# debbiemarkslab/EVcouplings

Measured on NVIDIA H100. Metric: PLM gradient evals/s as N*L^2*q cell-ops/s, higher is better.
Workload: dtype f32 parameters/accumulation; tensor-core products as bf16 hi+lo pairs (16 mantissa bits)

## Files before the change

### evcouplings_b200/_lib.py

```python
import ctypes
import os

_HERE = os.path.dirname(os.path.abspath(__file__))
LIB_PATH = os.path.join(_HERE, "csrc", "libevcplm.so")
ABI_VERSION = 2


class EngineUnavailableError(RuntimeError):
    """libevcplm.so (the sm_90a CUDA engine) is missing / unloadable / has no device."""


class EngineError(RuntimeError):
    """A libevcplm call returned non-zero."""


c_void_p = ctypes.c_void_p
c_i32 = ctypes.c_int32
c_i64 = ctypes.c_int64
c_f32 = ctypes.c_float
c_f64 = ctypes.c_double


class FitParams(ctypes.Structure):
    _fields_ = [("max_iterations", c_i32), ("m", c_i32), ("epsilon", c_f32), ("lambda_h", c_f32),
                ("lambda_J", c_f32), ("max_linesearch", c_i32), ("min_step", c_f64), ("max_step", c_f64),
                ("ftol", c_f64), ("gtol", c_f64), ("xtol", c_f64), ("precision_schedule", c_i32),
                ("switch_factor", c_f32)]


class FitResult(ctypes.Structure):
    _fields_ = [("status", c_i32), ("iterations", c_i32), ("evaluations", c_i32), ("switched_at", c_i32),
                ("fx", c_f64), ("negloglk", c_f64), ("seconds", c_f64)]


class FitState(ctypes.Structure):
    _fields_ = [("version", c_i32), ("returning", c_i32), ("status", c_i32), ("k", c_i32), ("evaluations", c_i32),
                ("m", c_i32), ("hist", c_i32), ("end", c_i32), ("low", c_i32), ("switched_at", c_i32),
                ("n", c_i64), ("fx", c_f64), ("negloglk", c_f64), ("xnorm", c_f64), ("gnorm", c_f64),
                ("ys", c_f64 * 32), ("yy", c_f64), ("seconds", c_f64)]


FIT_STATE_VERSION = 1
FIT_VEC_X, FIT_VEC_G, FIT_VEC_S, FIT_VEC_Y = 0, 1, 2, 3

ALLREDUCE_CB = ctypes.CFUNCTYPE(ctypes.c_int, ctypes.c_void_p, ctypes.c_void_p, c_i64, ctypes.c_void_p)
PROGRESS_CB = ctypes.CFUNCTYPE(ctypes.c_int, ctypes.c_void_p, c_i32, c_f64, c_f64, c_f64, c_f64, c_i32, c_f64,
                               c_f64, c_f64)
CHECKPOINT_CB = ctypes.CFUNCTYPE(ctypes.c_int, ctypes.c_void_p, ctypes.POINTER(FitState), ctypes.c_void_p)

LBFGS_STATUS = {
    0: "LBFGS_SUCCESS", 2: "LBFGS_ALREADY_MINIMIZED", -1021: "LBFGSERR_CANCELED",
    -1000: "LBFGSERR_INVALIDPARAMETERS", -1001: "LBFGSERR_MINIMUMSTEP", -1002: "LBFGSERR_MAXIMUMSTEP",
    -1003: "LBFGSERR_MAXIMUMLINESEARCH", -1004: "LBFGSERR_MAXIMUMITERATION", -1005: "LBFGSERR_WIDTHTOOSMALL",
    -1006: "LBFGSERR_ROUNDING_ERROR", -1007: "LBFGSERR_INCREASEGRADIENT",
}

PROTOTYPES = {
    "evc_abi_version": (ctypes.c_int, []),
    "evc_last_error": (ctypes.c_char_p, []),
    "evc_device_count": (ctypes.c_int, []),
    "evc_device_info": (ctypes.c_int, [c_i32, c_void_p, c_void_p, c_void_p, c_void_p]),
    "evc_hamming_counts": (ctypes.c_int, [c_void_p, c_i64, c_i32, c_i32, c_i32, c_void_p]),
    "evc_hamming_plane_words": (c_i64, [c_i64, c_i32]),
    "evc_hamming_num_tiles": (c_i64, [c_i64]),
    "evc_hamming_pack": (ctypes.c_int, [c_void_p, c_i64, c_i32, c_void_p, c_void_p]),
    "evc_hamming_count_tiles": (ctypes.c_int, [c_void_p, c_i64, c_i32, c_i32, c_i64, c_i64, c_void_p, c_void_p]),
    "evc_hamming_counts_mult": (ctypes.c_int, [c_void_p, c_void_p, c_i64, c_i32, c_i32, c_i32, c_void_p]),
    "evc_hamming_count_tiles_mult": (ctypes.c_int, [c_void_p, c_void_p, c_i64, c_i32, c_i32, c_i64, c_i64, c_void_p,
                                                    c_void_p]),
    "evc_msa_unique": (ctypes.c_int, [c_void_p, c_i64, c_i32, c_void_p, c_void_p, c_void_p, c_void_p, c_void_p]),
    "evc_msa_unique_host": (ctypes.c_int, [c_void_p, c_i64, c_i32, c_i32, c_void_p, c_void_p, c_void_p, c_void_p]),
    "evc_a2m_scan": (ctypes.c_int, [ctypes.c_char_p, c_void_p, c_void_p, c_void_p]),
    "evc_a2m_read": (ctypes.c_int, [ctypes.c_char_p, c_i64, c_i64, c_void_p, c_void_p, c_i64]),
    "evc_msa_encode": (ctypes.c_int, [c_void_p, c_i64, c_i64, c_void_p, c_void_p, c_i64, c_void_p, c_void_p, c_void_p]),
    "evc_identities_to_seq": (ctypes.c_int, [c_void_p, c_void_p, c_i64, c_i32, c_void_p, c_void_p]),
    "evc_plm_create": (ctypes.c_int, [c_void_p, c_void_p, c_i64, c_i32, c_i32, c_i32, c_void_p, c_i32]),
    "evc_plm_create_alphabet": (ctypes.c_int, [c_void_p, c_void_p, c_i64, c_i32, c_i32, c_i32, c_void_p, c_i32]),
    "evc_plm_destroy": (None, [c_void_p]),
    "evc_plm_num_params": (c_i64, [c_void_p]),
    "evc_plm_eval_data": (ctypes.c_int, [c_void_p, c_void_p, c_void_p, c_void_p, c_void_p]),
    "evc_plm_set_backward": (ctypes.c_int, [c_void_p, c_i32]),
    "evc_plm_set_forward": (ctypes.c_int, [c_void_p, c_i32]),
    "evc_plm_set_precision": (ctypes.c_int, [c_void_p, c_i32]),
    "evc_plm_set_seq_chunk": (ctypes.c_int, [c_void_p, c_i64]),
    "evc_plm_tc_bytes": (ctypes.c_int, [c_i64, c_i32, c_i32, c_i32, c_i64, c_i32, c_void_p]),
    "evc_plm_tc_bytes_alphabet": (ctypes.c_int, [c_i64, c_i32, c_i32, c_i32, c_i64, c_i32, c_void_p]),
    "evc_plm_device_bytes": (c_i64, [c_void_p]),
    "evc_fit_workspace_bytes": (c_i64, [c_i64, c_i32]),
    "evc_plm_set_host_history": (ctypes.c_int, [c_void_p, c_i32]),
    "evc_fit_workspace_split_bytes": (ctypes.c_int, [c_i64, c_i32, c_i32, c_void_p, c_void_p]),
    "evc_plm_host_bytes": (ctypes.c_int, [c_void_p, c_void_p, c_void_p]),
    "evc_fit_default_params": (None, [c_void_p]),
    "evc_plm_fit": (ctypes.c_int, [c_void_p, c_void_p, c_void_p, c_void_p, c_void_p, c_void_p, c_void_p, c_void_p,
                                   c_void_p]),
    "evc_plm_fit_checkpointed": (ctypes.c_int, [c_void_p, c_void_p, c_void_p, c_void_p, c_void_p, c_void_p, c_void_p,
                                                c_void_p, c_void_p, c_f64, c_void_p, c_void_p, c_void_p]),
    "evc_plm_fit_prepare": (ctypes.c_int, [c_void_p, c_i32]),
    "evc_plm_fit_vector": (ctypes.c_int, [c_void_p, c_i32, c_i32, c_void_p]),
    "evc_plm_pack_fx": (ctypes.c_int, [c_void_p, c_void_p, c_void_p]),
    "evc_plm_unpack_fx": (ctypes.c_int, [c_void_p, c_void_p, c_void_p]),
    "evc_plm_set_profiling": (ctypes.c_int, [c_void_p, c_i32]),
    "evc_plm_last_stage_ms": (ctypes.c_int, [c_void_p, c_void_p]),
    "evc_plm_add_regulariser": (ctypes.c_int, [c_void_p, c_void_p, c_void_p, c_void_p, c_f32, c_f32, c_void_p]),
    "evc_plm_eval_host": (ctypes.c_int, [c_void_p, c_void_p, c_void_p, c_void_p, c_f32, c_f32]),
    "evc_plm_weighted_counts": (ctypes.c_int, [c_void_p, c_void_p, c_void_p, c_void_p]),
    "evc_vec_dot": (ctypes.c_int, [c_void_p, c_void_p, c_i64, c_void_p, c_void_p]),
    "evc_vec_axpby": (ctypes.c_int, [c_void_p, c_void_p, c_f32, c_f32, c_i64, c_void_p]),
    "evc_vec_copy": (ctypes.c_int, [c_void_p, c_void_p, c_i64, c_void_p]),
    "evc_vec_sub": (ctypes.c_int, [c_void_p, c_void_p, c_void_p, c_i64, c_void_p]),
    "evc_vec_checksum": (ctypes.c_int, [c_void_p, c_i64, c_void_p, c_void_p]),
    "evc_lbfgs_direction": (ctypes.c_int, [c_void_p, c_void_p, c_void_p, c_void_p, c_void_p, c_void_p,
                                           c_i64, c_i32, c_i32, c_i32, c_void_p]),
    "evc_lbfgs_update_pair": (ctypes.c_int, [c_void_p, c_void_p, c_void_p, c_void_p, c_void_p, c_void_p,
                                             c_void_p, c_void_p, c_i64, c_void_p]),
    "evc_ec_scores": (ctypes.c_int, [c_void_p, c_void_p, c_void_p, c_i32, c_i32, c_void_p, c_void_p, c_void_p, c_void_p]),
    "evc_plm_energies": (ctypes.c_int, [c_void_p, c_void_p, c_void_p, c_void_p]),
    "evc_fn_scores": (ctypes.c_int, [c_void_p, c_i32, c_i32, c_void_p, c_void_p]),
}

_lib = None


def load():
    global _lib
    if _lib is not None:
        return _lib
    if not os.path.exists(LIB_PATH):
        raise EngineUnavailableError(
            "CUDA engine library not built: %s is missing. There is no CPU fallback; "
            "build it with evcouplings_b200/csrc/build.sh (nvcc, sm_90a)." % LIB_PATH)
    try:
        lib = ctypes.CDLL(LIB_PATH)
    except OSError as e:
        raise EngineUnavailableError("cannot load %s: %s" % (LIB_PATH, e))
    for name, (restype, argtypes) in PROTOTYPES.items():
        try:
            fn = getattr(lib, name)
        except AttributeError:
            raise EngineUnavailableError("%s does not export %s" % (LIB_PATH, name))
        fn.restype = restype
        fn.argtypes = argtypes
    if lib.evc_abi_version() != ABI_VERSION:
        raise EngineUnavailableError("libevcplm ABI version mismatch")
    _lib = lib
    return lib


def check(rc, what=""):
    if rc != 0:
        msg = load().evc_last_error()
        raise EngineError("%s failed: %s" % (what or "libevcplm call", msg.decode() if msg else "unknown error"))


def require_device():
    lib = load()
    n = lib.evc_device_count()
    if n <= 0:
        raise EngineUnavailableError(
            "libevcplm found no CUDA device; the PLM engine has no CPU fallback")
    return n
```

### evcouplings_b200/csrc/api.cu

```cuda
#include "../../include/evcplm.h"

#include <stdlib.h>

#include <algorithm>
#include <new>
#include <string>
#include <vector>

#include "common.cuh"
#include "internal.h"

namespace evc {
static thread_local std::string g_err;
void set_error(const std::string &msg) { g_err = msg; }
}

using namespace evc;

static cudaStream_t as_stream(void *s) { return reinterpret_cast<cudaStream_t>(s); }

static const char SUPPORTED_Q[] =
    "supported: 2 <= q <= 32 states with the gap as a state, 2 <= q <= 31 with the ignored gap coded q; "
    "every code must be below 32, the 5 bit-planes of the Hamming pass";

static int require_gather_q(const evc_plm *h, const char *what)
{
    if (plm_gather_supported_q(h->g.q)) return 0;
    set_error(std::string(what) + ": the gather kernels support q in {4, 5, 20, 21} only, this handle has q=" +
              std::to_string(h->g.q) + "; select the tensor-core path with evc_plm_set_forward(h, 1)");
    return 1;
}

static void plm_geom_init(PlmGeom &g, int64_t N, int L, int q, int gap_code)
{
    g.N = N;
    g.L = L;
    g.Lp = (int)round_up(L, 4);
    g.q = q;
    g.gap_code = gap_code;
    g.QB = gap_code >= 0 ? q + 1 : q;
    g.S = (q % 2) ? q : q + 1;
    g.Nr = round_up(N, PLM_BWD_TS);
    g.Nld = round_up(N, 32);
    g.L4 = g.Lp / 4;
    g.ntiles_f = (int)ceil_div(N, PLM_FWD_TS);
    g.ntiles_b = (int)ceil_div(N, PLM_BWD_TS);
    g.n_params = (int64_t)L * q + (int64_t)L * (L - 1) / 2 * q * q;
}
struct HandleBytes {
    size_t codes, msa4, wts;
    explicit HandleBytes(const PlmGeom &g)
        : codes((size_t)g.N * g.L), msa4((size_t)g.L4 * g.Nld * sizeof(uint32_t)), wts((size_t)g.N * sizeof(float)) {}
};
struct TcBwdBytes {
    size_t xt, rt, gd;
    explicit TcBwdBytes(const PlmTcGeom &t)
        : xt((size_t)t.Mp * t.Kp * 2), rt((size_t)t.Np * t.Kp * 2), gd((size_t)t.planes * t.Mp * t.Np * sizeof(float)) {}
};
struct TcFwdBytes {
    size_t x, wt, zt, gh_part, fx_part;
    TcFwdBytes(const PlmGeom &g, const PlmTcfGeom &t)
        : x((size_t)t.Xrows * t.Kw * 2), wt((size_t)t.Mp * t.Kw * 2), zt((size_t)t.Mp * t.Ns * sizeof(float)),
          gh_part((size_t)g.L * t.ntiles_s * g.S * sizeof(float)), fx_part((size_t)g.L * t.ntiles_s * sizeof(double)) {}
};

template <class T>
static bool dalloc(evc_plm *h, T **p, size_t bytes)
{
    if (cudaMalloc(p, bytes) != cudaSuccess) return false;
    h->bytes += (int64_t)bytes;
    return true;
}

extern "C" {

int evc_abi_version(void) { return EVCPLM_ABI_VERSION; }

const char *evc_last_error(void) { return g_err.c_str(); }

int evc_device_count(void)
{
    int n = 0;
    if (cudaGetDeviceCount(&n) != cudaSuccess) {
        set_error("cudaGetDeviceCount failed (no CUDA device / driver?)");
        return -1;
    }
    return n;
}

int evc_device_info(int32_t device, int32_t *sm_count, int32_t *cc_major, int32_t *cc_minor,
                    int64_t *total_mem_bytes)
{
    cudaDeviceProp p;
    EVC_CUDA(cudaGetDeviceProperties(&p, device));
    if (sm_count) *sm_count = p.multiProcessorCount;
    if (cc_major) *cc_major = p.major;
    if (cc_minor) *cc_minor = p.minor;
    if (total_mem_bytes) *total_mem_bytes = (int64_t)p.totalGlobalMem;
    return 0;
}

int64_t evc_hamming_plane_words(int64_t N, int32_t L) { return hamming_plane_words(N, L); }
int64_t evc_hamming_num_tiles(int64_t N) { return hamming_num_tiles(N); }

int evc_hamming_pack(const uint8_t *d_codes, int64_t N, int32_t L, uint32_t *d_planes, void *stream)
{
    return hamming_pack(d_codes, N, L, d_planes, as_stream(stream));
}

int evc_hamming_count_tiles(const uint32_t *d_planes, int64_t N, int32_t L, int32_t min_identical,
                            int64_t tile_begin, int64_t tile_end, int32_t *d_counts, void *stream)
{
    return hamming_count_tiles(d_planes, nullptr, N, L, min_identical, tile_begin, tile_end, d_counts,
                               as_stream(stream));
}

int evc_hamming_count_tiles_mult(const uint32_t *d_planes, const int32_t *d_mult, int64_t N, int32_t L,
                                 int32_t min_identical, int64_t tile_begin, int64_t tile_end, int32_t *d_counts,
                                 void *stream)
{
    if (!d_mult) { set_error("evc_hamming_count_tiles_mult: null multiplicities"); return 1; }
    return hamming_count_tiles(d_planes, d_mult, N, L, min_identical, tile_begin, tile_end, d_counts,
                               as_stream(stream));
}

static int hamming_counts_host(const char *fn, const uint8_t *codes, const int32_t *mult, int64_t N, int32_t L,
                               int32_t min_identical, int32_t device, int32_t *counts_out)
{
    const std::string name(fn);
    if (!codes || !counts_out || N <= 0 || L <= 0) {
        set_error(name + ": empty alignment or null pointer");
        return 1;
    }
    {
        unsigned mx = 0;
        const size_t total = (size_t)N * L;
        for (size_t e = 0; e < total; e++) mx = codes[e] > mx ? codes[e] : mx;
        if (mx >= 32) {
            set_error(name + ": sequence code " + std::to_string(mx) + " out of range (codes must be < 32)");
            return 1;
        }
    }
    if (mult) {
        int64_t sum = 0;
        for (int64_t r = 0; r < N; r++) {
            if (mult[r] < 1) { set_error(name + ": multiplicities must be >= 1"); return 1; }
            sum += mult[r];
        }
        if (sum > INT32_MAX) { set_error(name + ": the multiplicities sum to more than 2^31 - 1"); return 1; }
    }
    EVC_CUDA(cudaSetDevice(device));
    uint8_t *d_codes = nullptr;
    uint32_t *d_planes = nullptr;
    int32_t *d_counts = nullptr, *d_mult = nullptr;
    int rc = 1;
    do {
        if (cudaMalloc(&d_codes, (size_t)N * L) != cudaSuccess ||
            cudaMalloc(&d_planes, (size_t)hamming_plane_words(N, L) * sizeof(uint32_t)) != cudaSuccess ||
            cudaMalloc(&d_counts, (size_t)N * sizeof(int32_t)) != cudaSuccess ||
            (mult && cudaMalloc(&d_mult, (size_t)N * sizeof(int32_t)) != cudaSuccess)) {
            set_error(name + ": device allocation failed");
            break;
        }
        if (cudaMemcpy(d_codes, codes, (size_t)N * L, cudaMemcpyHostToDevice) != cudaSuccess ||
            (mult && cudaMemcpy(d_mult, mult, (size_t)N * sizeof(int32_t), cudaMemcpyHostToDevice) != cudaSuccess) ||
            cudaMemset(d_counts, 0, (size_t)N * sizeof(int32_t)) != cudaSuccess) {
            set_error(name + ": H2D failed");
            break;
        }
        if (hamming_pack(d_codes, N, L, d_planes, 0)) break;
        if (hamming_count_tiles(d_planes, d_mult, N, L, min_identical, 0, hamming_num_tiles(N), d_counts, 0)) break;
        if (cudaMemcpy(counts_out, d_counts, (size_t)N * sizeof(int32_t), cudaMemcpyDeviceToHost) !=
            cudaSuccess) {
            set_error(name + ": kernel/D2H failed: " + cudaGetErrorString(cudaGetLastError()));
            break;
        }
        rc = 0;
    } while (0);
    cudaFree(d_codes);
    cudaFree(d_planes);
    cudaFree(d_counts);
    cudaFree(d_mult);
    return rc;
}

int evc_hamming_counts(const uint8_t *codes, int64_t N, int32_t L, int32_t min_identical, int32_t device,
                       int32_t *counts_out)
{
    return hamming_counts_host("evc_hamming_counts", codes, nullptr, N, L, min_identical, device, counts_out);
}

int evc_hamming_counts_mult(const uint8_t *codes, const int32_t *mult, int64_t N, int32_t L, int32_t min_identical,
                            int32_t device, int32_t *counts_out)
{
    if (!mult) { set_error("evc_hamming_counts_mult: null multiplicities"); return 1; }
    return hamming_counts_host("evc_hamming_counts_mult", codes, mult, N, L, min_identical, device, counts_out);
}

int evc_msa_unique(const uint8_t *d_codes, int64_t N, int32_t L, int32_t *d_first, int32_t *d_inverse,
                   int32_t *d_mult, int64_t *U_out, void *stream)
{
    if (!d_codes || !d_first || !d_inverse || !d_mult || !U_out) {
        set_error("evc_msa_unique: null pointer");
        return 1;
    }
    return msa_unique(d_codes, N, L, d_first, d_inverse, d_mult, U_out, as_stream(stream));
}

int evc_msa_unique_host(const uint8_t *codes, int64_t N, int32_t L, int32_t device, int32_t *first_out,
                        int32_t *inverse_out, int32_t *mult_out, int64_t *U_out)
{
    if (!codes || !first_out || !inverse_out || !mult_out || !U_out || N <= 0 || L <= 0) {
        set_error("evc_msa_unique_host: empty alignment or null pointer");
        return 1;
    }
    EVC_CUDA(cudaSetDevice(device));
    uint8_t *d_codes = nullptr;
    int32_t *d_idx = nullptr;
    int rc = 1;
    do {
        if (cudaMalloc(&d_codes, (size_t)N * L) != cudaSuccess ||
            cudaMalloc(&d_idx, (size_t)3 * N * sizeof(int32_t)) != cudaSuccess) {
            set_error("evc_msa_unique_host: device allocation failed");
            break;
        }
        if (cudaMemcpy(d_codes, codes, (size_t)N * L, cudaMemcpyHostToDevice) != cudaSuccess) {
            set_error("evc_msa_unique_host: H2D failed");
            break;
        }
        int64_t U = 0;
        if (msa_unique(d_codes, N, L, d_idx, d_idx + N, d_idx + 2 * N, &U, 0)) break;
        if (cudaMemcpy(first_out, d_idx, (size_t)U * sizeof(int32_t), cudaMemcpyDeviceToHost) != cudaSuccess ||
            cudaMemcpy(inverse_out, d_idx + N, (size_t)N * sizeof(int32_t), cudaMemcpyDeviceToHost) != cudaSuccess ||
            cudaMemcpy(mult_out, d_idx + 2 * N, (size_t)U * sizeof(int32_t), cudaMemcpyDeviceToHost) != cudaSuccess) {
            set_error(std::string("evc_msa_unique_host: D2H failed: ") + cudaGetErrorString(cudaGetLastError()));
            break;
        }
        *U_out = U;
        rc = 0;
    } while (0);
    cudaFree(d_codes);
    cudaFree(d_idx);
    return rc;
}

int evc_identities_to_seq(const uint8_t *d_codes, const uint8_t *d_seq, int64_t N, int32_t L, int32_t *d_out,
                          void *stream)
{
    if (!d_codes || !d_seq || !d_out) { set_error("evc_identities_to_seq: null pointer"); return 1; }
    return identities_to_seq(d_codes, d_seq, N, L, d_out, as_stream(stream));
}

void evc_plm_destroy(evc_plm_t *h)
{
    if (!h) return;
    cudaSetDevice(h->device);
    cudaFree(h->d_codes);
    cudaFree(h->d_msa4);
    cudaFree(h->d_perm);
    cudaFree(h->d_bstart);
    cudaFree(h->d_wts);
    cudaFree(h->d_W);
    cudaFree(h->d_G);
    cudaFree(h->d_R);
    cudaFree(h->d_gh_part);
    cudaFree(h->d_fx_part);
    cudaFree(h->d_x_tmp);
    cudaFree(h->d_g_tmp);
    cudaFree(h->d_fx_tmp);
    cudaFree(h->d_xt);
    cudaFree(h->d_rt_hi);
    cudaFree(h->d_rt_lo);
    cudaFree(h->d_Gd);
    free(h->tc_maps);
    cudaFree(h->d_x1h);
    cudaFree(h->d_wt_hi);
    cudaFree(h->d_wt_lo);
    cudaFree(h->d_zt);
    cudaFree(h->d_gh_part2);
    cudaFree(h->d_fx_part2);
    free(h->tcf_maps);
    cudaFree(h->d_wp_hi);
    cudaFree(h->d_wp_lo);
    cudaFree(h->d_gh_part3);
    cudaFree(h->d_fx_part3);
    free(h->tcff_maps);
    for (int k = 0; k < 6; k++)
        if (h->ev[k]) cudaEventDestroy(h->ev[k]);
    fit_work_free(h->fit);
    delete h;
}

static int plm_create(const char *fn, bool any_q, evc_plm_t **out, const uint8_t *codes, int64_t N, int32_t L,
                      int32_t q, int32_t gap_code, const float *weights, int32_t device)
{
    const std::string name(fn);
    if (!out || !codes || !weights) { set_error(name + ": null pointer"); return 1; }
    *out = nullptr;
    if (N <= 0 || L < 2) { set_error(name + ": need N >= 1 sequences and L >= 2 sites"); return 1; }
    if (!any_q && !plm_gather_supported_q(q)) {
        set_error(name + ": unsupported number of states q=" + std::to_string(q) +
                  " (supported: 4, 5, 20, 21; evc_plm_create_alphabet takes 2 <= q <= 32)");
        return 1;
    }
    if (gap_code >= 0 && gap_code != q) {
        set_error(name + ": gap_code must be -1 or q");
        return 1;
    }
    if (!plm_supported_q(q, gap_code)) {
        set_error(name + ": unsupported number of states q=" + std::to_string(q) +
                  (gap_code >= 0 ? " with the ignored gap" : "") + " (" + SUPPORTED_Q + ")");
        return 1;
    }
    if (L > 65535) { set_error(name + ": L too large"); return 1; }
    {
        unsigned mx = 0;
        const size_t total = (size_t)N * L;
        for (size_t e = 0; e < total; e++) mx = codes[e] > mx ? codes[e] : mx;
        if ((int)mx >= (gap_code >= 0 ? q + 1 : q)) {
            set_error(name + ": sequence code " + std::to_string(mx) + " out of range (valid: 0.." +
                      std::to_string((gap_code >= 0 ? q + 1 : q) - 1) + (gap_code >= 0 ? ", the last one being the ignored gap)" : ")"));
            return 1;
        }
    }
    EVC_CUDA(cudaSetDevice(device));
    evc_plm *h = new (std::nothrow) evc_plm();
    if (!h) { set_error(name + ": out of host memory"); return 1; }
    h->device = device;
    PlmGeom &g = h->g;
    plm_geom_init(g, N, L, q, gap_code);
    const HandleBytes hb(g);

    bool ok = dalloc(h, &h->d_codes, hb.codes) && dalloc(h, &h->d_msa4, hb.msa4) && dalloc(h, &h->d_wts, hb.wts);
    if (!ok) {
        set_error(name + ": device allocation failed: " +
                  cudaGetErrorString(cudaGetLastError()));
        evc_plm_destroy(h);
        return 1;
    }
    ok = cudaMemcpy(h->d_codes, codes, (size_t)N * L, cudaMemcpyHostToDevice) == cudaSuccess &&
         cudaMemcpy(h->d_wts, weights, (size_t)N * sizeof(float), cudaMemcpyHostToDevice) == cudaSuccess;
    if (!ok || plm_pack_msa(g, h->d_codes, h->d_msa4, 0) || cudaDeviceSynchronize() != cudaSuccess) {
        if (ok) set_error(name + ": packing failed: " + cudaGetErrorString(cudaGetLastError()));
        else set_error(name + ": H2D failed");
        evc_plm_destroy(h);
        return 1;
    }
    *out = h;
    return 0;
}

int evc_plm_create(evc_plm_t **out, const uint8_t *codes, int64_t N, int32_t L, int32_t q, int32_t gap_code,
                   const float *weights, int32_t device)
{
    return plm_create("evc_plm_create", false, out, codes, N, L, q, gap_code, weights, device);
}

int evc_plm_create_alphabet(evc_plm_t **out, const uint8_t *codes, int64_t N, int32_t L, int32_t q, int32_t gap_code,
                            const float *weights, int32_t device)
{
    return plm_create("evc_plm_create_alphabet", true, out, codes, N, L, q, gap_code, weights, device);
}

static int ensure_expanded(evc_plm *h)
{
    if (h->expanded_ready) return 0;
    EVC_CUDA(cudaSetDevice(h->device));
    const PlmGeom &g = h->g;
    const size_t w_bytes = (size_t)g.w_floats() * sizeof(float);
    const size_t r_bytes = (size_t)g.L * g.Nr * g.S * sizeof(float);
    if (!dalloc(h, &h->d_W, w_bytes) || !dalloc(h, &h->d_R, r_bytes)) {
        set_error(std::string("libevcplm: device allocation of the expanded couplings failed: ") +
                  cudaGetErrorString(cudaGetLastError()));
        return 1;
    }
    EVC_CUDA(cudaMemset(h->d_W, 0, w_bytes));
    EVC_CUDA(cudaMemset(h->d_R, 0, r_bytes));
    h->expanded_ready = true;
    return 0;
}

static int ensure_gather(evc_plm *h)
{
    if (h->gather_ready) return 0;
    if (require_gather_q(h, "libevcplm")) return 1;
    if (ensure_expanded(h)) return 1;
    const PlmGeom &g = h->g;
    const size_t w_bytes = (size_t)g.w_floats() * sizeof(float);
    const bool ok = dalloc(h, &h->d_perm, (size_t)g.ntiles_b * g.L * PLM_BWD_CAP * sizeof(uint32_t)) &&
                    dalloc(h, &h->d_bstart, (size_t)g.ntiles_b * g.L * PLM_BWD_BS * sizeof(uint16_t)) &&
                    dalloc(h, &h->d_G, w_bytes) &&
                    dalloc(h, &h->d_gh_part, (size_t)g.L * g.ntiles_f * g.S * sizeof(float)) &&
                    dalloc(h, &h->d_fx_part, (size_t)g.L * g.ntiles_f * sizeof(double));
    if (!ok) {
        set_error(std::string("libevcplm: device allocation of the gather-path buffers failed: ") +
                  cudaGetErrorString(cudaGetLastError()));
        return 1;
    }
    if (plm_build_buckets(g, h->d_codes, h->d_perm, h->d_bstart, 0)) return 1;
    EVC_CUDA(cudaDeviceSynchronize());
    h->gather_ready = true;
    return 0;
}

int64_t evc_plm_num_params(const evc_plm_t *h) { return h ? h->g.n_params : -1; }

int evc_plm_set_precision(evc_plm_t *h, int32_t mode)
{
    if (!h) { set_error("evc_plm_set_precision: null handle"); return 1; }
    if (mode != 0 && mode != 1) {
        set_error("evc_plm_set_precision: mode must be 0 (fp32-equivalent, bf16 hi+lo products) or 1 (bf16 tiles)");
        return 1;
    }
    h->precision = mode;
    return 0;
}

int evc_plm_eval_data(evc_plm_t *h, const float *d_x, float *d_g, double *d_fx, void *stream)
{
    if (!h || !d_x || !d_g || !d_fx) { set_error("evc_plm_eval_data: null pointer"); return 1; }
    cudaStream_t st = as_stream(stream);
    const PlmGeom &g = h->g;
    const bool prof = h->profiling;
    const bool tc = h->bwd_mode == 1;
    const bool tcf = h->fwd_mode == 1;
    const bool tcff = h->fwd_mode == 2;
    const int single = h->precision == 1 ? 1 : 0;
    void *rt_lo = single ? nullptr : h->d_rt_lo;
    float *gJ = d_g + (int64_t)g.L * g.q;
    if (tc && h->tc.n_chunks > 1) {
        if (!tcf) {
            set_error("evc_plm_eval_data: sequence chunks need the tensor-core forward (evc_plm_set_forward 1)");
            return 1;
        }
        h->ev_valid = false;
        if (plm_tcf_expand(g, h->tcf, d_x, h->d_wt_hi, h->d_wt_lo, single, st)) return 1;
        for (int c = 0; c < h->tc.n_chunks; c++) {
            const int64_t n0 = (int64_t)c * h->tc.C, nreal = std::min(h->tc.C, g.N - n0);
            if (plm_tcf_build_x(g, h->tcf, h->d_msa4, h->d_x1h, n0, st)) return 1;
            if (plm_tc_build_xt(g, h->tc, h->d_msa4, h->d_xt, n0, st)) return 1;
            if (plm_tcf_logits(g, h->tcf, h->tcf_maps, h->d_zt, single, nreal, st)) return 1;
            if (plm_tcf_softmax(g, h->tcf, h->d_zt, d_x, h->d_msa4, h->d_wts, h->d_rt_hi, rt_lo, h->tc.Kp,
                                h->d_gh_part2, h->d_fx_part2, n0, nreal, st))
                return 1;
            if (plm_tc_backward(g, h->tc, h->tc_maps, h->d_Gd, single, c, st)) return 1;
        }
        if (plm_tc_finalize_pairs(g, h->tc, h->d_Gd, h->tc.planes, gJ, 1.0f, st)) return 1;
        return plm_finalize_fields_n(g, h->d_gh_part2, h->d_fx_part2, d_g, d_fx, h->tcf.ntiles_s, st);
    }
    if (!tc || (!tcf && !tcff)) {
        if (require_gather_q(h, "evc_plm_eval_data") || ensure_gather(h)) return 1;
    }
    if (prof) EVC_CUDA(cudaEventRecord(h->ev[0], st));
    if (tcff) {
        if (plm_tcff_expand(g, h->tcff, d_x, h->d_wp_hi, h->d_wp_lo, single, st)) return 1;
        if (prof) EVC_CUDA(cudaEventRecord(h->ev[1], st));
        if (plm_tcff_forward(g, h->tcff, h->tcff_maps, d_x, h->d_msa4, h->d_wts, h->d_rt_hi, h->d_rt_lo, h->tc.Kp,
                             h->d_gh_part3, h->d_fx_part3, single, st))
            return 1;
        if (prof) {
            EVC_CUDA(cudaEventRecord(h->ev[2], st));
            EVC_CUDA(cudaEventRecord(h->ev[3], st));
        }
        if (plm_tc_backward(g, h->tc, h->tc_maps, h->d_Gd, single, 0, st)) return 1;
        if (prof) EVC_CUDA(cudaEventRecord(h->ev[4], st));
        if (plm_tc_finalize_pairs(g, h->tc, h->d_Gd, h->tc.planes, gJ, 1.0f, st)) return 1;
        if (plm_finalize_fields_n(g, h->d_gh_part3, h->d_fx_part3, d_g, d_fx, h->tcff.ntile_part, st)) return 1;
    } else if (tcf) {
        if (plm_tcf_expand(g, h->tcf, d_x, h->d_wt_hi, h->d_wt_lo, single, st)) return 1;
        if (prof) EVC_CUDA(cudaEventRecord(h->ev[1], st));
        if (plm_tcf_logits(g, h->tcf, h->tcf_maps, h->d_zt, single, g.N, st)) return 1;
        if (prof) EVC_CUDA(cudaEventRecord(h->ev[2], st));
        if (plm_tcf_softmax(g, h->tcf, h->d_zt, d_x, h->d_msa4, h->d_wts, h->d_rt_hi, rt_lo, h->tc.Kp,
                            h->d_gh_part2, h->d_fx_part2, 0, g.N, st))
            return 1;
        if (prof) EVC_CUDA(cudaEventRecord(h->ev[3], st));
        if (plm_tc_backward(g, h->tc, h->tc_maps, h->d_Gd, single, 0, st)) return 1;
        if (prof) EVC_CUDA(cudaEventRecord(h->ev[4], st));
        if (plm_tc_finalize_pairs(g, h->tc, h->d_Gd, h->tc.planes, gJ, 1.0f, st)) return 1;
        if (plm_finalize_fields_n(g, h->d_gh_part2, h->d_fx_part2, d_g, d_fx, h->tcf.ntiles_s, st)) return 1;
    } else {
        if (plm_expand(g, d_x, h->d_W, st)) return 1;
        if (!tc) EVC_CUDA(cudaMemsetAsync(h->d_G, 0, (size_t)g.w_floats() * sizeof(float), st));
        if (prof) EVC_CUDA(cudaEventRecord(h->ev[1], st));
        if (plm_forward(g, h->d_W, d_x, h->d_msa4, h->d_wts, h->d_R, tc ? h->d_rt_hi : nullptr,
                        tc ? h->d_rt_lo : nullptr, h->tc.Kp, h->d_gh_part, h->d_fx_part, st))
            return 1;
        if (prof) {
            EVC_CUDA(cudaEventRecord(h->ev[2], st));
            EVC_CUDA(cudaEventRecord(h->ev[3], st));
        }
        if (tc) {
            if (plm_tc_backward(g, h->tc, h->tc_maps, h->d_Gd, single, 0, st)) return 1;
            if (prof) EVC_CUDA(cudaEventRecord(h->ev[4], st));
            if (plm_tc_finalize_pairs(g, h->tc, h->d_Gd, h->tc.planes, gJ, 1.0f, st)) return 1;
            if (plm_finalize_fields(g, h->d_gh_part, h->d_fx_part, d_g, d_fx, st)) return 1;
        } else {
            if (plm_backward(g, h->d_R, h->d_perm, h->d_bstart, h->d_G, st)) return 1;
            if (prof) EVC_CUDA(cudaEventRecord(h->ev[4], st));
            if (plm_finalize(g, h->d_G, h->d_gh_part, h->d_fx_part, d_g, gJ, d_fx, 1.0f, st)) return 1;
        }
    }
    if (prof) {
        EVC_CUDA(cudaEventRecord(h->ev[5], st));
        h->ev_valid = true;
    }
    return 0;
}

int evc_plm_set_backward(evc_plm_t *h, int32_t mode)
{
    if (!h) { set_error("evc_plm_set_backward: null handle"); return 1; }
    if (mode != 0 && mode != 1) { set_error("evc_plm_set_backward: mode must be 0 (gather) or 1 (tensor core)"); return 1; }
    if (mode == 0 && require_gather_q(h, "evc_plm_set_backward")) return 1;
    EVC_CUDA(cudaSetDevice(h->device));
    if (mode == 1 && !h->d_xt) {
        int sm_count = 0;
        EVC_CUDA(cudaDeviceGetAttribute(&sm_count, cudaDevAttrMultiProcessorCount, h->device));
        plm_tc_geometry(h->g, sm_count, h->seq_chunk, h->tc);
        const PlmTcGeom &t = h->tc;
        const TcBwdBytes b(t);
        if (!dalloc(h, &h->d_xt, b.xt) || !dalloc(h, &h->d_rt_hi, b.rt) || !dalloc(h, &h->d_rt_lo, b.rt) ||
            !dalloc(h, &h->d_Gd, b.gd)) {
            set_error(std::string("evc_plm_set_backward: device allocation failed: ") +
                      cudaGetErrorString(cudaGetLastError()));
            return 1;
        }
        EVC_CUDA(cudaMemset(h->d_xt, 0, b.xt));
        EVC_CUDA(cudaMemset(h->d_rt_hi, 0, b.rt));
        EVC_CUDA(cudaMemset(h->d_rt_lo, 0, b.rt));
        EVC_CUDA(cudaMemset(h->d_Gd, 0, b.gd));
        if (t.n_chunks == 1 && plm_tc_build_xt(h->g, t, h->d_msa4, h->d_xt, 0, 0)) return 1;
        EVC_CUDA(cudaDeviceSynchronize());
        h->tc_maps = aligned_alloc(64, round_up((int64_t)plm_tc_map_bytes(), 64));
        if (!h->tc_maps) { set_error("evc_plm_set_backward: out of host memory"); return 1; }
        if (plm_tc_make_maps(t, h->d_xt, h->d_rt_hi, h->d_rt_lo, h->tc_maps)) return 1;
    }
    h->bwd_mode = mode;
    return 0;
}

int evc_plm_set_forward(evc_plm_t *h, int32_t mode)
{
    if (!h) { set_error("evc_plm_set_forward: null handle"); return 1; }
    if (mode < 0 || mode > 2) {
        set_error("evc_plm_set_forward: mode must be 0 (gather), 1 (tensor core) or 2 (tensor core, fused softmax)");
        return 1;
    }
    if (mode == 0 && require_gather_q(h, "evc_plm_set_forward")) return 1;
    EVC_CUDA(cudaSetDevice(h->device));
    const int64_t chunk = plm_seq_chunk_round(h->seq_chunk);
    const bool chunked = chunk > 0 && chunk < h->g.N;
    if (mode == 2 && (!plm_tcff_supported(h->g) || (int64_t)h->g.L * h->g.q > 8192 || chunked)) mode = 1;
    if (mode >= 1) {
        if (evc_plm_set_backward(h, 1)) return 1;
        if (!h->d_x1h) {
            plm_tcf_geometry(h->g, h->tc, h->tcf);
            const PlmTcfGeom &t = h->tcf;
            const TcFwdBytes b(h->g, t);
            if (!dalloc(h, &h->d_x1h, b.x)) {
                set_error("evc_plm_set_forward: device allocation failed (one-hot operand)");
                return 1;
            }
            EVC_CUDA(cudaMemset(h->d_x1h, 0, b.x));
            if (h->tc.n_chunks == 1 && plm_tcf_build_x(h->g, t, h->d_msa4, h->d_x1h, 0, 0)) return 1;
            EVC_CUDA(cudaDeviceSynchronize());
        }
    }
    if (mode == 1 && !h->d_zt) {
        const PlmTcfGeom &t = h->tcf;
        const TcFwdBytes b(h->g, t);
        if (!dalloc(h, &h->d_wt_hi, b.wt) || !dalloc(h, &h->d_wt_lo, b.wt) || !dalloc(h, &h->d_zt, b.zt) ||
            !dalloc(h, &h->d_gh_part2, b.gh_part) || !dalloc(h, &h->d_fx_part2, b.fx_part)) {
            set_error(std::string("evc_plm_set_forward: device allocation failed: ") +
                      cudaGetErrorString(cudaGetLastError()));
            return 1;
        }
        EVC_CUDA(cudaMemset(h->d_wt_hi, 0, b.wt));
        EVC_CUDA(cudaMemset(h->d_wt_lo, 0, b.wt));
        h->tcf_maps = aligned_alloc(64, round_up((int64_t)plm_tc_map_bytes(), 64));
        if (!h->tcf_maps) { set_error("evc_plm_set_forward: out of host memory"); return 1; }
        if (plm_tcf_make_maps(t, h->d_wt_hi, h->d_wt_lo, h->d_x1h, h->tcf_maps)) return 1;
    }
    if (mode == 2 && !h->d_wp_hi) {
        plm_tcff_geometry(h->g, h->tcff);
        const PlmTcffGeom &t = h->tcff;
        const size_t wb = (size_t)t.Np * t.Kw * 2;
        if (!dalloc(h, &h->d_wp_hi, wb) || !dalloc(h, &h->d_wp_lo, wb) ||
            !dalloc(h, &h->d_gh_part3, (size_t)h->g.L * t.ntile_part * h->g.S * sizeof(float)) ||
            !dalloc(h, &h->d_fx_part3, (size_t)h->g.L * t.ntile_part * sizeof(double))) {
            set_error(std::string("evc_plm_set_forward: device allocation failed: ") +
                      cudaGetErrorString(cudaGetLastError()));
            return 1;
        }
        EVC_CUDA(cudaMemset(h->d_wp_hi, 0, wb));
        EVC_CUDA(cudaMemset(h->d_wp_lo, 0, wb));
        h->tcff_maps = aligned_alloc(64, round_up((int64_t)plm_tc_map_bytes(), 64));
        if (!h->tcff_maps) { set_error("evc_plm_set_forward: out of host memory"); return 1; }
        if (plm_tcff_make_maps(t, h->d_x1h, h->d_wp_hi, h->d_wp_lo, h->tcff_maps)) return 1;
    }
    h->fwd_mode = mode;
    return 0;
}

int evc_plm_set_seq_chunk(evc_plm_t *h, int64_t seq_chunk)
{
    if (!h) { set_error("evc_plm_set_seq_chunk: null handle"); return 1; }
    if (seq_chunk < 0) { set_error("evc_plm_set_seq_chunk: seq_chunk must be >= 0 (0: whole shard)"); return 1; }
    const int64_t c = plm_seq_chunk_round(seq_chunk);
    if (h->d_xt) {
        const int64_t have = h->tc.n_chunks > 1 ? h->tc.C : 0;
        const int64_t want = (c > 0 && c < h->g.N) ? c : 0;
        if (have != want) {
            set_error("evc_plm_set_seq_chunk: the tensor-core buffers already exist for " +
                      (have ? std::to_string(have) + " sequences per chunk" : std::string("the whole shard")) +
                      "; set the chunk before evc_plm_set_backward / evc_plm_set_forward");
            return 1;
        }
    }
    h->seq_chunk = c;
    return 0;
}

static int plm_tc_bytes(const char *fn, bool any_q, int64_t N, int32_t L, int32_t q, int32_t gap_code,
                        int64_t seq_chunk, int32_t sm_count, int64_t *bytes_out)
{
    const std::string name(fn);
    if (!bytes_out) { set_error(name + ": null pointer"); return 1; }
    const bool q_ok = any_q ? plm_supported_q(q, gap_code) : plm_gather_supported_q(q);
    if (N <= 0 || L < 2 || L > 65535 || !q_ok || (gap_code >= 0 && gap_code != q) || seq_chunk < 0 ||
        sm_count <= 0) {
        set_error(name + ": invalid arguments (need N >= 1, 2 <= L <= 65535, gap_code -1 or q, seq_chunk >= 0, "
                  "sm_count >= 1; q: " + (any_q ? std::string(SUPPORTED_Q)
                                                : std::string("4, 5, 20 or 21; evc_plm_tc_bytes_alphabet takes "
                                                              "2 <= q <= 32")) + ")");
        return 1;
    }
    PlmGeom g{};
    plm_geom_init(g, N, L, q, gap_code);
    PlmTcGeom t{};
    plm_tc_geometry(g, sm_count, seq_chunk, t);
    PlmTcfGeom f{};
    plm_tcf_geometry(g, t, f);
    const HandleBytes hb(g);
    const TcBwdBytes bb(t);
    const TcFwdBytes fb(g, f);
    *bytes_out = (int64_t)(hb.codes + hb.msa4 + hb.wts + bb.xt + 2 * bb.rt + bb.gd + fb.x + 2 * fb.wt + fb.zt +
                           fb.gh_part + fb.fx_part);
    return 0;
}

int evc_plm_tc_bytes(int64_t N, int32_t L, int32_t q, int32_t gap_code, int64_t seq_chunk, int32_t sm_count,
                     int64_t *bytes_out)
{
    return plm_tc_bytes("evc_plm_tc_bytes", false, N, L, q, gap_code, seq_chunk, sm_count, bytes_out);
}

int evc_plm_tc_bytes_alphabet(int64_t N, int32_t L, int32_t q, int32_t gap_code, int64_t seq_chunk,
                              int32_t sm_count, int64_t *bytes_out)
{
    return plm_tc_bytes("evc_plm_tc_bytes_alphabet", true, N, L, q, gap_code, seq_chunk, sm_count, bytes_out);
}

int64_t evc_plm_device_bytes(const evc_plm_t *h) { return h ? h->bytes + fit_work_bytes(h->fit) : -1; }

int64_t evc_fit_workspace_bytes(int64_t n, int32_t m) { return n > 0 && m > 0 ? fit_work_bytes(n, m) : -1; }

int evc_fit_workspace_split_bytes(int64_t n, int32_t m, int32_t host_pairs, int64_t *device_bytes,
                                  int64_t *host_bytes)
{
    if (!device_bytes || !host_bytes) { set_error("evc_fit_workspace_split_bytes: null pointer"); return 1; }
    if (n <= 0 || m < 1 || m > 32 || host_pairs < 0 || host_pairs > m) {
        set_error("evc_fit_workspace_split_bytes: invalid arguments (need n >= 1, 1 <= m <= 32, "
                  "0 <= host_pairs <= m)");
        return 1;
    }
    fit_work_bytes(n, m, host_pairs, device_bytes, host_bytes);
    return 0;
}

int evc_plm_set_host_history(evc_plm_t *h, int32_t host_pairs)
{
    if (!h) { set_error("evc_plm_set_host_history: null handle"); return 1; }
    if (host_pairs < 0 || host_pairs > 32) {
        set_error("evc_plm_set_host_history: host_pairs must be in 0..32");
        return 1;
    }
    h->host_pairs = host_pairs;
    return 0;
}

int evc_plm_host_bytes(const evc_plm_t *h, int64_t *bytes_out, double *pin_seconds_out)
{
    if (!h || !bytes_out) { set_error("evc_plm_host_bytes: null pointer"); return 1; }
    *bytes_out = fit_work_host_bytes(h->fit);
    if (pin_seconds_out) *pin_seconds_out = fit_work_pin_seconds(h->fit);
    return 0;
}

int evc_plm_set_profiling(evc_plm_t *h, int32_t enable)
{
    if (!h) { set_error("evc_plm_set_profiling: null handle"); return 1; }
    EVC_CUDA(cudaSetDevice(h->device));
    if (enable && !h->ev[0])
        for (int k = 0; k < 6; k++) EVC_CUDA(cudaEventCreate(&h->ev[k]));
    h->profiling = enable != 0;
    h->ev_valid = false;
    return 0;
}

int evc_plm_last_stage_ms(evc_plm_t *h, float *ms_out)
{
    if (!h || !ms_out) { set_error("evc_plm_last_stage_ms: null pointer"); return 1; }
    if (h->bwd_mode == 1 && h->tc.n_chunks > 1) {
        set_error("evc_plm_last_stage_ms: per-stage timing is not recorded when the sequences are processed in "
                  "chunks (evc_plm_set_seq_chunk); time the whole evaluation instead");
        return 1;
    }
    if (!h->ev_valid) { set_error("evc_plm_last_stage_ms: no profiled evaluation recorded"); return 1; }
    EVC_CUDA(cudaEventSynchronize(h->ev[5]));
    for (int k = 0; k < 5; k++) EVC_CUDA(cudaEventElapsedTime(&ms_out[k], h->ev[k], h->ev[k + 1]));
    return 0;
}

int evc_plm_add_regulariser(evc_plm_t *h, const float *d_x, float *d_g, double *d_fx, float lambda_h,
                            float lambda_J, void *stream)
{
    if (!h || !d_x || !d_g || !d_fx) { set_error("evc_plm_add_regulariser: null pointer"); return 1; }
    return plm_add_reg(h->g, d_x, d_g, d_fx, lambda_h, lambda_J, as_stream(stream));
}

int evc_plm_eval_host(evc_plm_t *h, const float *x, float *gout, double *fx_out, float lambda_h,
                      float lambda_J)
{
    if (!h || !x || !gout || !fx_out) { set_error("evc_plm_eval_host: null pointer"); return 1; }
    EVC_CUDA(cudaSetDevice(h->device));
    const size_t nb = (size_t)h->g.n_params * sizeof(float);
    if (!h->d_x_tmp) {
        if (!dalloc(h, &h->d_x_tmp, nb) || !dalloc(h, &h->d_g_tmp, nb) || !dalloc(h, &h->d_fx_tmp, 2 * sizeof(double))) {
            set_error("evc_plm_eval_host: device allocation failed");
            return 1;
        }
    }
    EVC_CUDA(cudaMemcpyAsync(h->d_x_tmp, x, nb, cudaMemcpyHostToDevice, 0));
    if (evc_plm_eval_data(h, h->d_x_tmp, h->d_g_tmp, h->d_fx_tmp, nullptr)) return 1;
    if (evc_plm_add_regulariser(h, h->d_x_tmp, h->d_g_tmp, h->d_fx_tmp, lambda_h, lambda_J, nullptr)) return 1;
    EVC_CUDA(cudaMemcpyAsync(gout, h->d_g_tmp, nb, cudaMemcpyDeviceToHost, 0));
    EVC_CUDA(cudaMemcpyAsync(fx_out, h->d_fx_tmp, 2 * sizeof(double), cudaMemcpyDeviceToHost, 0));
    EVC_CUDA(cudaStreamSynchronize(0));
    return 0;
}

int evc_plm_weighted_counts(evc_plm_t *h, float *d_fi_counts, float *d_fij_counts, void *stream)
{
    if (!h || !d_fi_counts || !d_fij_counts) { set_error("evc_plm_weighted_counts: null pointer"); return 1; }
    cudaStream_t st = as_stream(stream);
    const PlmGeom &g = h->g;
    if (h->bwd_mode == 1 && h->d_gh_part2) {
        const int ntiles = h->tcf.ntiles_s;
        const PlmTcGeom &t = h->tc;
        for (int c = 0; c < t.n_chunks; c++) {
            const int64_t n0 = (int64_t)c * t.C, nreal = std::min(t.C, g.N - n0);
            if (t.n_chunks > 1 && plm_tc_build_xt(g, t, h->d_msa4, h->d_xt, n0, st)) return 1;
            if (plm_tc_onehot_residual(g, ntiles, h->d_msa4, h->d_wts, h->d_rt_hi, h->d_rt_lo, t.Kp, h->d_gh_part2,
                                       h->d_fx_part2, n0, nreal, st))
                return 1;
            if (plm_tc_backward(g, t, h->tc_maps, h->d_Gd, 0, c, st)) return 1;
        }
        if (plm_tc_finalize_pairs(g, t, h->d_Gd, t.planes, d_fij_counts, 0.5f, st)) return 1;
        return plm_finalize_fields_n(g, h->d_gh_part2, nullptr, d_fi_counts, nullptr, ntiles, st);
    }
    if (require_gather_q(h, "evc_plm_weighted_counts") || ensure_gather(h)) return 1;
    EVC_CUDA(cudaMemsetAsync(h->d_G, 0, (size_t)g.w_floats() * sizeof(float), st));
    if (plm_onehot_residual(g, h->d_msa4, h->d_wts, h->d_R, h->d_gh_part, st)) return 1;
    if (plm_backward(g, h->d_R, h->d_perm, h->d_bstart, h->d_G, st)) return 1;
    return plm_finalize(g, h->d_G, h->d_gh_part, nullptr, d_fi_counts, d_fij_counts, nullptr, 0.5f, st);
}

int evc_ec_scores(const float *d_J_tri, const float *d_fij_tri, const float *d_fi, int32_t L, int32_t q,
                  float *d_fn_raw, float *d_fn_zero_sum, float *d_mi, void *stream)
{
    if (!d_J_tri) { set_error("evc_ec_scores: null pointer"); return 1; }
    return ec_scores(d_J_tri, d_fij_tri, d_fi, L, q, d_fn_raw, d_fn_zero_sum, d_mi, as_stream(stream));
}

int evc_plm_energies(evc_plm_t *h, const float *d_x, double *d_out, void *stream)
{
    if (!h || !d_x || !d_out) { set_error("evc_plm_energies: null pointer"); return 1; }
    cudaStream_t st = as_stream(stream);
    const PlmGeom &g = h->g;
    if (ensure_expanded(h)) return 1;
    if (plm_expand(g, d_x, h->d_W, st)) return 1;
    return plm_energies(g, h->d_W, d_x, h->d_msa4, h->d_R, d_out, st);
}

int evc_vec_dot(const float *d_a, const float *d_b, int64_t n, double *d_out, void *stream)
{
    return vec_dot(d_a, d_b, n, d_out, as_stream(stream));
}
int evc_vec_axpby(float *d_y, const float *d_x, float a, float b, int64_t n, void *stream)
{
    return vec_axpby(d_y, d_x, a, b, n, as_stream(stream));
}
int evc_vec_copy(float *d_dst, const float *d_src, int64_t n, void *stream)
{
    EVC_CUDA(cudaMemcpyAsync(d_dst, d_src, (size_t)n * sizeof(float), cudaMemcpyDeviceToDevice,
                             as_stream(stream)));
    return 0;
}
int evc_vec_sub(float *d_out, const float *d_a, const float *d_b, int64_t n, void *stream)
{
    return vec_sub(d_out, d_a, d_b, n, as_stream(stream));
}
int evc_vec_checksum(const float *d_v, int64_t n, uint64_t *d_out, void *stream)
{
    return vec_checksum(d_v, n, d_out, as_stream(stream));
}
int evc_lbfgs_direction(float *d_d, const float *d_g, const float *d_S, const float *d_Y, const double *d_ys,
                        double *d_scratch, int64_t n, int32_t m, int32_t bound, int32_t end, void *stream)
{
    return lbfgs_direction(d_d, d_g, d_S, d_Y, d_ys, d_scratch, n, m, bound, end, as_stream(stream));
}
int evc_lbfgs_update_pair(float *d_S_slot, float *d_Y_slot, const float *d_x, const float *d_xp,
                          const float *d_g, const float *d_gp, double *d_ys_slot, double *d_yy, int64_t n,
                          void *stream)
{
    return lbfgs_update_pair(d_S_slot, d_Y_slot, d_x, d_xp, d_g, d_gp, d_ys_slot, d_yy, n, as_stream(stream));
}
int evc_fn_scores(const float *d_J_tri, int32_t L, int32_t q, float *d_fn, void *stream)
{
    return fn_scores(d_J_tri, L, q, d_fn, as_stream(stream));
}

}
```

### evcouplings_b200/csrc/internal.h

```cpp
#pragma once
#include <cuda_runtime.h>
#include <stdint.h>

namespace evc {

int64_t hamming_plane_words(int64_t N, int L);
int64_t hamming_num_tiles(int64_t N);
int hamming_pack(const uint8_t *d_codes, int64_t N, int L, uint32_t *d_planes, cudaStream_t st);
int hamming_count_tiles(const uint32_t *d_planes, const int *d_mult, int64_t N, int L, int min_identical,
                        int64_t tile_begin, int64_t tile_end, int *d_counts, cudaStream_t st);

int identities_to_seq(const uint8_t *d_codes, const uint8_t *d_seq, int64_t N, int L, int *d_out, cudaStream_t st);

int msa_unique(const uint8_t *d_codes, int64_t N, int L, int *d_first, int *d_inverse, int *d_mult, int64_t *U_out,
               cudaStream_t st);

struct PlmGeom {
    int64_t N;
    int L;
    int Lp;
    int q;
    int QB;
    int S;
    int gap_code;
    int64_t Nr;
    int64_t Nld;
    int L4;
    int ntiles_f;
    int ntiles_b;
    int64_t n_params;
    __host__ __device__ int64_t blk() const { return (int64_t)QB * S; }
    __host__ __device__ int64_t row_block() const { return (int64_t)Lp * blk(); }
    __host__ __device__ int64_t w_floats() const { return (int64_t)L * row_block(); }
};

constexpr int PLM_FWD_TS = 512;
constexpr int PLM_BWD_TS = 2048;
constexpr int PLM_BWD_CAP = 2224;
constexpr int PLM_BWD_BS = 24;

constexpr int PLM_MAX_Q = 32;
bool plm_supported_q(int q, int gap_code);
bool plm_gather_supported_q(int q);
int plm_pack_msa(const PlmGeom &g, const uint8_t *d_codes, uint32_t *d_msa4, cudaStream_t st);
int plm_build_buckets(const PlmGeom &g, const uint8_t *d_codes, uint32_t *d_perm, uint16_t *d_bstart,
                      cudaStream_t st);
int plm_expand(const PlmGeom &g, const float *d_x, float *d_W, cudaStream_t st);
int plm_forward(const PlmGeom &g, const float *d_W, const float *d_x, const uint32_t *d_msa4,
                const float *d_wts, float *d_R, void *d_rt_hi, void *d_rt_lo, int64_t Kp, float *d_gh_part,
                double *d_fx_part, cudaStream_t st);
int plm_onehot_residual(const PlmGeom &g, const uint32_t *d_msa4, const float *d_wts, float *d_R,
                        float *d_gh_part, cudaStream_t st);
int plm_backward(const PlmGeom &g, const float *d_R, const uint32_t *d_perm, const uint16_t *d_bstart,
                 float *d_G, cudaStream_t st);
int plm_finalize(const PlmGeom &g, const float *d_G, const float *d_gh_part, const double *d_fx_part,
                 float *d_gh, float *d_gJ, double *d_fx, float scale_pair, cudaStream_t st);
int plm_add_reg(const PlmGeom &g, const float *d_x, float *d_g, double *d_fx, float lambda_h,
                float lambda_J, cudaStream_t st);

constexpr int64_t PLM_SEQ_CHUNK_ALIGN = 768;
int64_t plm_seq_chunk_round(int64_t seq_chunk);
struct PlmTcGeom {
    int64_t C;
    int n_chunks;
    int64_t Mp;
    int64_t Np;
    int64_t Kp;
    int ksplit;
    int ksplit_last;
    int planes;
    int64_t kp_chunk(int c, int64_t N) const
    {
        const int64_t n = N - (int64_t)c * C < C ? N - (int64_t)c * C : C;
        return (n + 63) / 64 * 64;
    }
};
void plm_tc_geometry(const PlmGeom &g, int sm_count, int64_t seq_chunk, PlmTcGeom &t);
size_t plm_tc_map_bytes();
int plm_tc_build_xt(const PlmGeom &g, const PlmTcGeom &t, const uint32_t *d_msa4, void *d_xt, int64_t n0,
                    cudaStream_t st);
int plm_tc_make_maps(const PlmTcGeom &t, void *d_xt, void *d_rt_hi, void *d_rt_lo, void *maps_out_host);
int plm_tc_backward(const PlmGeom &g, const PlmTcGeom &t, const void *maps_host, float *d_Gd, int single, int chunk,
                    cudaStream_t st);
int plm_tc_onehot_residual(const PlmGeom &g, int ntiles, const uint32_t *d_msa4, const float *d_wts, void *d_rt_hi,
                           void *d_rt_lo, int64_t Kp, float *d_gh_part, double *d_fx_part, int64_t n0, int64_t nreal,
                           cudaStream_t st);
int plm_tc_finalize_pairs(const PlmGeom &g, const PlmTcGeom &t, const float *d_Gd, int planes, float *d_gJ,
                          float scale, cudaStream_t st);
struct PlmTcfGeom {
    int64_t Mp;
    int64_t Kw;
    int64_t Ns;
    int64_t Xrows;
    int ntiles_s;
};
void plm_tcf_geometry(const PlmGeom &g, const PlmTcGeom &tc, PlmTcfGeom &t);
int plm_tcf_build_x(const PlmGeom &g, const PlmTcfGeom &t, const uint32_t *d_msa4, void *d_x1h, int64_t n0,
                    cudaStream_t st);
int plm_tcf_make_maps(const PlmTcfGeom &t, void *d_wt_hi, void *d_wt_lo, void *d_x1h, void *maps_out_host);
int plm_tcf_expand(const PlmGeom &g, const PlmTcfGeom &t, const float *d_x, void *d_wt_hi, void *d_wt_lo,
                   int single, cudaStream_t st);
int plm_tcf_logits(const PlmGeom &g, const PlmTcfGeom &t, const void *maps_host, float *d_zt, int single,
                   int64_t nreal, cudaStream_t st);
int plm_tcf_softmax(const PlmGeom &g, const PlmTcfGeom &t, const float *d_zt, const float *d_x,
                    const uint32_t *d_msa4, const float *d_wts, void *d_rt_hi, void *d_rt_lo, int64_t Kp,
                    float *d_gh_part, double *d_fx_part, int64_t n0, int64_t nreal, cudaStream_t st);
struct PlmTcffGeom {
    int n_tiles;
    int m_tiles;
    int64_t Np;
    int64_t Kw;
    int64_t Xrows;
    int ntile_part;
};
void plm_tcff_geometry(const PlmGeom &g, PlmTcffGeom &t);
bool plm_tcff_supported(const PlmGeom &g);
int plm_tcff_make_maps(const PlmTcffGeom &t, void *d_x1h, void *d_wp_hi, void *d_wp_lo, void *maps_out_host);
int plm_tcff_expand(const PlmGeom &g, const PlmTcffGeom &t, const float *d_x, void *d_wp_hi, void *d_wp_lo,
                    int single, cudaStream_t st);
int plm_tcff_forward(const PlmGeom &g, const PlmTcffGeom &t, const void *maps_host, const float *d_x,
                     const uint32_t *d_msa4, const float *d_wts, void *d_rt_hi, void *d_rt_lo, int64_t Kp,
                     float *d_gh_part, double *d_fx_part, int single, cudaStream_t st);
int plm_finalize_fields_n(const PlmGeom &g, const float *d_gh_part, const double *d_fx_part, float *d_gh,
                          double *d_fx, int ntiles, cudaStream_t st);
int plm_finalize_fields(const PlmGeom &g, const float *d_gh_part, const double *d_fx_part, float *d_gh,
                        double *d_fx, cudaStream_t st);

int ec_scores(const float *d_J, const float *d_fij, const float *d_fi, int L, int q, float *d_fn_raw,
              float *d_fn_zs, float *d_mi, cudaStream_t st);
int plm_energies(const PlmGeom &g, const float *d_W, const float *d_x, const uint32_t *d_msa4, float *d_epart,
                 double *d_out, cudaStream_t st);

int vec_dot(const float *a, const float *b, int64_t n, double *out, cudaStream_t st);
int vec_axpby(float *y, const float *x, float a, float b, int64_t n, cudaStream_t st);
int vec_sub(float *out, const float *a, const float *b, int64_t n, cudaStream_t st);
int vec_checksum(const float *v, int64_t n, uint64_t *out, cudaStream_t st);
int lbfgs_direction(float *d, const float *g, const float *S, const float *Y, const double *ys,
                    double *scratch, int64_t n, int m, int bound, int end, cudaStream_t st);
int lbfgs_update_pair(float *s, float *y, const float *x, const float *xp, const float *g,
                      const float *gp, double *ys, double *yy, int64_t n, cudaStream_t st);
int fn_scores(const float *J, int L, int q, float *fn, cudaStream_t st);

struct FitWork;
void fit_work_free(FitWork *w);
int64_t fit_work_bytes(int64_t n, int m);
void fit_work_bytes(int64_t n, int m, int host_pairs, int64_t *device_bytes, int64_t *host_bytes);
int64_t fit_work_bytes(const FitWork *w);
int64_t fit_work_host_bytes(const FitWork *w);
double fit_work_pin_seconds(const FitWork *w);

}

struct evc_plm {
    int device = 0;
    evc::PlmGeom g{};
    uint8_t *d_codes = nullptr;
    uint32_t *d_msa4 = nullptr;
    float *d_wts = nullptr;
    bool expanded_ready = false;
    bool gather_ready = false;
    uint32_t *d_perm = nullptr;
    uint16_t *d_bstart = nullptr;
    float *d_W = nullptr;
    float *d_G = nullptr;
    float *d_R = nullptr;
    float *d_gh_part = nullptr;
    double *d_fx_part = nullptr;
    float *d_x_tmp = nullptr;
    float *d_g_tmp = nullptr;
    double *d_fx_tmp = nullptr;
    int precision = 0;
    int bwd_mode = 0;
    evc::PlmTcGeom tc{};
    void *d_xt = nullptr;
    void *d_rt_hi = nullptr;
    void *d_rt_lo = nullptr;
    float *d_Gd = nullptr;
    void *tc_maps = nullptr;
    int fwd_mode = 0;
    evc::PlmTcfGeom tcf{};
    void *d_x1h = nullptr;
    void *d_wt_hi = nullptr;
    void *d_wt_lo = nullptr;
    float *d_zt = nullptr;
    float *d_gh_part2 = nullptr;
    double *d_fx_part2 = nullptr;
    void *tcf_maps = nullptr;
    evc::PlmTcffGeom tcff{};
    void *d_wp_hi = nullptr;
    void *d_wp_lo = nullptr;
    float *d_gh_part3 = nullptr;
    double *d_fx_part3 = nullptr;
    void *tcff_maps = nullptr;
    bool profiling = false;
    cudaEvent_t ev[6] = {nullptr, nullptr, nullptr, nullptr, nullptr, nullptr};
    bool ev_valid = false;
    evc::FitWork *fit = nullptr;
    int host_pairs = 0;
    int64_t seq_chunk = 0;
    int64_t bytes = 0;
};
```

### evcouplings_b200/csrc/plm_tc.cu

```cuda
#include <cuda.h>
#include <cuda_bf16.h>

#include <stdlib.h>

#include <algorithm>

#include "common.cuh"
#include "internal.h"

namespace evc {

constexpr int TC_BM = 128;
constexpr int TC_BN = 192;
constexpr int TC_BK = 64;
constexpr int TC_MAX_STAGES = 8;
constexpr int TC_A_BYTES = TC_BM * TC_BK * 2;
constexpr int TC_B_BYTES = TC_BN * TC_BK * 2;
constexpr int TC_SMEM_LIMIT = 232448;
constexpr int TC_SMEM_HEAD = 2048;
constexpr int TC_THREADS = 384;
constexpr int TC_CONSUMERS = 256;
constexpr int TC_K_CHUNK = 32;
constexpr int TC_MAX_KSPLIT = 8;
constexpr int TC_REG_PRODUCER = 40;
constexpr int TC_REG_CONSUMER = 232;

__device__ __forceinline__ void mbar_wait_bounded(uint64_t *bar, uint32_t parity)
{
    uint32_t done = 0;
    for (uint64_t it = 0; it < (1ull << 31); it++) {
        asm volatile(
            "{\n.reg .pred p;\n"
            "mbarrier.try_wait.parity.shared::cta.b64 p, [%1], %2;\n"
            "selp.u32 %0, 1, 0, p;\n}\n"
            : "=r"(done)
            : "r"(smem_u32(bar)), "r"(parity)
            : "memory");
        if (done) return;
    }
    __trap();
}

__device__ __forceinline__ void mbar_arrive(uint64_t *bar)
{
    asm volatile("mbarrier.arrive.shared::cta.b64 _, [%0];" ::"r"(smem_u32(bar)) : "memory");
}

__device__ __forceinline__ void tma_load_2d(void *smem_dst, const CUtensorMap *tmap, int c0, int c1, uint64_t *bar)
{
    asm volatile(
        "cp.async.bulk.tensor.2d.shared::cluster.global.mbarrier::complete_tx::bytes [%0], [%1, {%3, %4}], [%2];"
        ::"r"(smem_u32(smem_dst)), "l"(reinterpret_cast<uint64_t>(tmap)), "r"(smem_u32(bar)), "r"(c0), "r"(c1)
        : "memory");
}

__device__ __forceinline__ void tma_load_2d_hint(void *smem_dst, const CUtensorMap *tmap, int c0, int c1,
                                                 uint64_t *bar, uint64_t policy)
{
    asm volatile(
        "cp.async.bulk.tensor.2d.shared::cluster.global.mbarrier::complete_tx::bytes.L2::cache_hint "
        "[%0], [%1, {%3, %4}], [%2], %5;"
        ::"r"(smem_u32(smem_dst)), "l"(reinterpret_cast<uint64_t>(tmap)), "r"(smem_u32(bar)), "r"(c0), "r"(c1),
        "l"(policy)
        : "memory");
}
__device__ __forceinline__ uint64_t l2_policy_evict_last()
{
    uint64_t p;
    asm volatile("createpolicy.fractional.L2::evict_last.b64 %0, 1.0;" : "=l"(p));
    return p;
}

template <int N>
__device__ __forceinline__ void setmaxnreg_dec() { asm volatile("setmaxnreg.dec.sync.aligned.u32 %0;\n" ::"n"(N)); }
template <int N>
__device__ __forceinline__ void setmaxnreg_inc() { asm volatile("setmaxnreg.inc.sync.aligned.u32 %0;\n" ::"n"(N)); }

__device__ __forceinline__ void wgmma_fence() { asm volatile("wgmma.fence.sync.aligned;" ::: "memory"); }
__device__ __forceinline__ void wgmma_commit() { asm volatile("wgmma.commit_group.sync.aligned;" ::: "memory"); }
template <int N>
__device__ __forceinline__ void wgmma_wait() { asm volatile("wgmma.wait_group.sync.aligned %0;" ::"n"(N) : "memory"); }

template <int R>
__device__ __forceinline__ void fence_regs(float *d)
{
#pragma unroll
    for (int i = 0; i < R; i++) asm volatile("" : "+f"(d[i])::"memory");
}

__device__ __forceinline__ void consumer_sync() { asm volatile("bar.sync 1, %0;" ::"n"(TC_CONSUMERS) : "memory"); }

__device__ __forceinline__ uint64_t make_desc_sw128(const void *smem_ptr)
{
    const uint32_t addr = smem_u32(smem_ptr);
    uint64_t d = 0;
    d |= (uint64_t)((addr >> 4) & 0x3FFF);
    d |= (uint64_t)1 << 16;
    d |= (uint64_t)(1024 >> 4) << 32;
    d |= (uint64_t)1 << 62;
    return d;
}

template <int N>
__device__ __forceinline__ void wgmma_bf16(float *d, uint64_t da, uint64_t db, uint32_t scale_d);
template <>
__device__ __forceinline__ void wgmma_bf16<192>(float *d, uint64_t da, uint64_t db, uint32_t scale_d)
{
    asm volatile(
        "{\n.reg .pred p;\n"
        "setp.ne.b32 p, %98, 0;\n"
        "wgmma.mma_async.sync.aligned.m64n192k16.f32.bf16.bf16 "
        "{"
        "%0, %1, %2, %3, %4, %5, %6, %7, %8, %9, %10, %11, %12, %13, %14, %15, "
        "%16, %17, %18, %19, %20, %21, %22, %23, %24, %25, %26, %27, %28, %29, %30, %31, "
        "%32, %33, %34, %35, %36, %37, %38, %39, %40, %41, %42, %43, %44, %45, %46, %47, "
        "%48, %49, %50, %51, %52, %53, %54, %55, %56, %57, %58, %59, %60, %61, %62, %63, "
        "%64, %65, %66, %67, %68, %69, %70, %71, %72, %73, %74, %75, %76, %77, %78, %79, "
        "%80, %81, %82, %83, %84, %85, %86, %87, %88, %89, %90, %91, %92, %93, %94, %95"
        "}, %96, %97, p, 1, 1, 0, 0;\n}\n"
        : "+f"(d[0]), "+f"(d[1]), "+f"(d[2]), "+f"(d[3]), "+f"(d[4]), "+f"(d[5]), "+f"(d[6]), "+f"(d[7]),
          "+f"(d[8]), "+f"(d[9]), "+f"(d[10]), "+f"(d[11]), "+f"(d[12]), "+f"(d[13]), "+f"(d[14]), "+f"(d[15]),
          "+f"(d[16]), "+f"(d[17]), "+f"(d[18]), "+f"(d[19]), "+f"(d[20]), "+f"(d[21]), "+f"(d[22]), "+f"(d[23]),
          "+f"(d[24]), "+f"(d[25]), "+f"(d[26]), "+f"(d[27]), "+f"(d[28]), "+f"(d[29]), "+f"(d[30]), "+f"(d[31]),
          "+f"(d[32]), "+f"(d[33]), "+f"(d[34]), "+f"(d[35]), "+f"(d[36]), "+f"(d[37]), "+f"(d[38]), "+f"(d[39]),
          "+f"(d[40]), "+f"(d[41]), "+f"(d[42]), "+f"(d[43]), "+f"(d[44]), "+f"(d[45]), "+f"(d[46]), "+f"(d[47]),
          "+f"(d[48]), "+f"(d[49]), "+f"(d[50]), "+f"(d[51]), "+f"(d[52]), "+f"(d[53]), "+f"(d[54]), "+f"(d[55]),
          "+f"(d[56]), "+f"(d[57]), "+f"(d[58]), "+f"(d[59]), "+f"(d[60]), "+f"(d[61]), "+f"(d[62]), "+f"(d[63]),
          "+f"(d[64]), "+f"(d[65]), "+f"(d[66]), "+f"(d[67]), "+f"(d[68]), "+f"(d[69]), "+f"(d[70]), "+f"(d[71]),
          "+f"(d[72]), "+f"(d[73]), "+f"(d[74]), "+f"(d[75]), "+f"(d[76]), "+f"(d[77]), "+f"(d[78]), "+f"(d[79]),
          "+f"(d[80]), "+f"(d[81]), "+f"(d[82]), "+f"(d[83]), "+f"(d[84]), "+f"(d[85]), "+f"(d[86]), "+f"(d[87]),
          "+f"(d[88]), "+f"(d[89]), "+f"(d[90]), "+f"(d[91]), "+f"(d[92]), "+f"(d[93]), "+f"(d[94]), "+f"(d[95])
        : "l"(da), "l"(db), "r"(scale_d));
}
template <>
__device__ __forceinline__ void wgmma_bf16<176>(float *d, uint64_t da, uint64_t db, uint32_t scale_d)
{
    asm volatile(
        "{\n.reg .pred p;\n"
        "setp.ne.b32 p, %90, 0;\n"
        "wgmma.mma_async.sync.aligned.m64n176k16.f32.bf16.bf16 "
        "{"
        "%0, %1, %2, %3, %4, %5, %6, %7, %8, %9, %10, %11, %12, %13, %14, %15, "
        "%16, %17, %18, %19, %20, %21, %22, %23, %24, %25, %26, %27, %28, %29, %30, %31, "
        "%32, %33, %34, %35, %36, %37, %38, %39, %40, %41, %42, %43, %44, %45, %46, %47, "
        "%48, %49, %50, %51, %52, %53, %54, %55, %56, %57, %58, %59, %60, %61, %62, %63, "
        "%64, %65, %66, %67, %68, %69, %70, %71, %72, %73, %74, %75, %76, %77, %78, %79, "
        "%80, %81, %82, %83, %84, %85, %86, %87"
        "}, %88, %89, p, 1, 1, 0, 0;\n}\n"
        : "+f"(d[0]), "+f"(d[1]), "+f"(d[2]), "+f"(d[3]), "+f"(d[4]), "+f"(d[5]), "+f"(d[6]), "+f"(d[7]),
          "+f"(d[8]), "+f"(d[9]), "+f"(d[10]), "+f"(d[11]), "+f"(d[12]), "+f"(d[13]), "+f"(d[14]), "+f"(d[15]),
          "+f"(d[16]), "+f"(d[17]), "+f"(d[18]), "+f"(d[19]), "+f"(d[20]), "+f"(d[21]), "+f"(d[22]), "+f"(d[23]),
          "+f"(d[24]), "+f"(d[25]), "+f"(d[26]), "+f"(d[27]), "+f"(d[28]), "+f"(d[29]), "+f"(d[30]), "+f"(d[31]),
          "+f"(d[32]), "+f"(d[33]), "+f"(d[34]), "+f"(d[35]), "+f"(d[36]), "+f"(d[37]), "+f"(d[38]), "+f"(d[39]),
          "+f"(d[40]), "+f"(d[41]), "+f"(d[42]), "+f"(d[43]), "+f"(d[44]), "+f"(d[45]), "+f"(d[46]), "+f"(d[47]),
          "+f"(d[48]), "+f"(d[49]), "+f"(d[50]), "+f"(d[51]), "+f"(d[52]), "+f"(d[53]), "+f"(d[54]), "+f"(d[55]),
          "+f"(d[56]), "+f"(d[57]), "+f"(d[58]), "+f"(d[59]), "+f"(d[60]), "+f"(d[61]), "+f"(d[62]), "+f"(d[63]),
          "+f"(d[64]), "+f"(d[65]), "+f"(d[66]), "+f"(d[67]), "+f"(d[68]), "+f"(d[69]), "+f"(d[70]), "+f"(d[71]),
          "+f"(d[72]), "+f"(d[73]), "+f"(d[74]), "+f"(d[75]), "+f"(d[76]), "+f"(d[77]), "+f"(d[78]), "+f"(d[79]),
          "+f"(d[80]), "+f"(d[81]), "+f"(d[82]), "+f"(d[83]), "+f"(d[84]), "+f"(d[85]), "+f"(d[86]), "+f"(d[87])
        : "l"(da), "l"(db), "r"(scale_d));
}

template <int N>
__device__ __forceinline__ void wgmma_kblock(float *acc, uint64_t a, uint64_t b, uint64_t a2, uint64_t b2, bool two,
                                             bool overwrite)
{
#pragma unroll
    for (int k = 0; k < TC_BK / 16; k++) {
        const uint64_t koff = (uint64_t)((k * 16 * 2) >> 4);
        wgmma_bf16<N>(acc, a + koff, b + koff, (overwrite && k == 0) ? 0u : 1u);
        if (two) wgmma_bf16<N>(acc, a2 + koff, b2 + koff, 1u);
    }
}

template <int N>
__device__ __forceinline__ void tc_mainloop(float *acc, uint64_t *full, uint64_t *empty, int &s, uint32_t &ph,
                                            int n_stages, int stage_bytes, int kb0, int kb1, uint64_t desc0,
                                            uint64_t off_a, uint64_t off_b, uint64_t off_a2, uint64_t off_b2, bool two)
{
    int prev = -1;
    for (int kb = kb0; kb < kb1; kb++) {
        mbar_wait_bounded(&full[s], ph);
        wgmma_fence();
        const uint64_t d = desc0 + (uint64_t)((s * stage_bytes) >> 4);
        wgmma_kblock<N>(acc, d + off_a, d + off_b, d + off_a2, d + off_b2, two, kb == kb0);
        wgmma_commit();
        wgmma_wait<1>();
        if (prev >= 0) mbar_arrive(&empty[prev]);
        prev = s;
        if (++s == n_stages) { s = 0; ph ^= 1u; }
    }
    wgmma_wait<0>();
    fence_regs<N / 2>(acc);
    if (prev >= 0) mbar_arrive(&empty[prev]);
}

__device__ __forceinline__ void decode_tile(int tile, int m_tiles, int n_tiles, int mgroup, int &m_tile, int &n_tile)
{
    const int full = (m_tiles / mgroup) * mgroup * n_tiles;
    if (tile < full) {
        const int per = mgroup * n_tiles;
        const int g = tile / per, r = tile - g * per;
        n_tile = r / mgroup;
        m_tile = g * mgroup + (r - n_tile * mgroup);
    } else {
        const int rem = m_tiles % mgroup, r = tile - full;
        n_tile = r / rem;
        m_tile = (m_tiles / mgroup) * mgroup + (r - n_tile * rem);
    }
}

struct TcSmem {
    uint64_t *full, *empty;
    unsigned char *ring;
};
__device__ __forceinline__ TcSmem tc_smem_layout(unsigned char *smem_dyn)
{
    unsigned char *base = reinterpret_cast<unsigned char *>((reinterpret_cast<uintptr_t>(smem_dyn) + 1023) &
                                                            ~static_cast<uintptr_t>(1023));
    TcSmem l;
    l.full = reinterpret_cast<uint64_t *>(base);
    l.empty = l.full + TC_MAX_STAGES;
    l.ring = base + 1024;
    return l;
}
__device__ __forceinline__ void tc_init_barriers(const TcSmem &l, int n_stages)
{
    if (threadIdx.x == 0) {
        for (int s = 0; s < n_stages; s++) {
            mbar_init(&l.full[s], 1);
            mbar_init(&l.empty[s], TC_CONSUMERS);
        }
        mbar_fence_init();
    }
    __syncthreads();
}

template <int SPLIT_A, int SINGLE, int ACC = 0>
__global__ void __launch_bounds__(TC_THREADS, 1)
tc_gemm_kernel(const __grid_constant__ CUtensorMap tm0, const __grid_constant__ CUtensorMap tm1,
               const __grid_constant__ CUtensorMap tm2, float *__restrict__ D, int64_t ldd, int m_tiles, int n_tiles,
               int num_kb, int k_chunk, int mgroup, int n_stages, int ksplit, int64_t plane, int acc_planes)
{
    constexpr int BYTES0 = TC_A_BYTES;
    constexpr int BYTES1 = TC_B_BYTES;
    constexpr int BYTES2 = SPLIT_A ? TC_A_BYTES : TC_B_BYTES;
    constexpr int stage_bytes = BYTES0 + BYTES1 + (SINGLE ? 0 : BYTES2);
    extern __shared__ unsigned char smem_dyn[];
    const TcSmem l = tc_smem_layout(smem_dyn);
    const int tiles = m_tiles * n_tiles;
    const int slice = (int)blockIdx.x / tiles;
    int m_tile, n_tile;
    decode_tile((int)blockIdx.x - slice * tiles, m_tiles, n_tiles, mgroup, m_tile, n_tile);
    const int kb_per = (num_kb + ksplit - 1) / ksplit;
    const int kb_begin = slice * kb_per, kb_end = min(num_kb, kb_begin + kb_per);
    tc_init_barriers(l, n_stages);

    if (threadIdx.x < 128) {
        setmaxnreg_dec<TC_REG_PRODUCER>();
        if (threadIdx.x == 0) {
            const uint64_t keep = l2_policy_evict_last();
            int s = 0;
            uint32_t ph = 0;
            for (int kb = kb_begin; kb < kb_end; kb++) {
                mbar_wait_bounded(&l.empty[s], ph ^ 1u);
                unsigned char *st = l.ring + s * stage_bytes;
                mbar_expect_tx(&l.full[s], (uint32_t)stage_bytes);
                if (SPLIT_A) {
                    tma_load_2d_hint(st, &tm0, kb * TC_BK, m_tile * TC_BM, &l.full[s], keep);
                    tma_load_2d(st + BYTES0, &tm2, kb * TC_BK, n_tile * TC_BN, &l.full[s]);
                    if (!SINGLE) tma_load_2d_hint(st + BYTES0 + BYTES1, &tm1, kb * TC_BK, m_tile * TC_BM, &l.full[s], keep);
                } else {
                    tma_load_2d(st, &tm0, kb * TC_BK, m_tile * TC_BM, &l.full[s]);
                    tma_load_2d(st + BYTES0, &tm1, kb * TC_BK, n_tile * TC_BN, &l.full[s]);
                    if (!SINGLE) tma_load_2d(st + BYTES0 + BYTES1, &tm2, kb * TC_BK, n_tile * TC_BN, &l.full[s]);
                }
                if (++s == n_stages) { s = 0; ph ^= 1u; }
            }
        }
    } else {
        setmaxnreg_inc<TC_REG_CONSUMER>();
        const int cw = (threadIdx.x >> 7) - 1;
        constexpr uint64_t OFF1 = (uint64_t)(BYTES0 >> 4), OFF2 = (uint64_t)((BYTES0 + BYTES1) >> 4);
        const uint64_t arow = (uint64_t)((cw * 64 * TC_BK * 2) >> 4);
        const uint64_t desc0 = make_desc_sw128(l.ring);
        float acc[TC_BN / 2], sum[TC_BN / 2];
#pragma unroll
        for (int u = 0; u < TC_BN / 2; u++) acc[u] = 0.f;
        const int n_chunks = (kb_end - kb_begin + k_chunk - 1) / k_chunk;
        int s = 0;
        uint32_t ph = 0;
        for (int c = 0; c < n_chunks; c++) {
            const int kb0 = kb_begin + c * k_chunk, kb1 = min(kb_end, kb0 + k_chunk);
            if (SPLIT_A) tc_mainloop<TC_BN>(acc, l.full, l.empty, s, ph, n_stages, stage_bytes, kb0, kb1, desc0,
                                            arow, OFF1, OFF2 + arow, OFF1, !SINGLE);
            else tc_mainloop<TC_BN>(acc, l.full, l.empty, s, ph, n_stages, stage_bytes, kb0, kb1, desc0,
                                    arow, OFF1, arow, OFF2, !SINGLE);
#pragma unroll
            for (int u = 0; u < TC_BN / 2; u++) sum[u] = (c == 0) ? acc[u] : sum[u] + acc[u];
        }
        const int t = threadIdx.x & 127;
        const int64_t row = (int64_t)m_tile * TC_BM + cw * 64 + (t >> 5) * 16 + ((t & 31) >> 2);
        float *out = D + slice * plane + row * ldd + (int64_t)n_tile * TC_BN + 2 * (t & 3);
        if (ACC && slice < acc_planes) {
#pragma unroll
            for (int c8 = 0; c8 < TC_BN / 8; c8++) {
                float2 *p0 = reinterpret_cast<float2 *>(out + 8 * c8);
                float2 *p1 = reinterpret_cast<float2 *>(out + 8 * ldd + 8 * c8);
                const float2 v0 = __ldcs(p0), v1 = __ldcs(p1);
                __stcs(p0, make_float2(v0.x + sum[4 * c8], v0.y + sum[4 * c8 + 1]));
                __stcs(p1, make_float2(v1.x + sum[4 * c8 + 2], v1.y + sum[4 * c8 + 3]));
            }
            return;
        }
#pragma unroll
        for (int c8 = 0; c8 < TC_BN / 8; c8++) {
            __stcs(reinterpret_cast<float2 *>(out + 8 * c8), make_float2(sum[4 * c8], sum[4 * c8 + 1]));
            __stcs(reinterpret_cast<float2 *>(out + 8 * ldd + 8 * c8), make_float2(sum[4 * c8 + 2], sum[4 * c8 + 3]));
        }
    }
}

constexpr int TF_BN = 176;
constexpr int TF_SITES = 8;
constexpr int TF_B_BYTES = TF_BN * TC_BK * 2;
constexpr int TF_PITCH = TF_BN + 1;

template <int SINGLE>
__global__ void __launch_bounds__(TC_THREADS, 1)
tc_fwd_fused_kernel(const __grid_constant__ CUtensorMap tm_x, const __grid_constant__ CUtensorMap tm_whi,
                    const __grid_constant__ CUtensorMap tm_wlo, const float *__restrict__ h,
                    const uint32_t *__restrict__ msa4, const float *__restrict__ wts,
                    __nv_bfloat16 *__restrict__ Rt_hi, __nv_bfloat16 *__restrict__ Rt_lo, int64_t Kp,
                    float *__restrict__ gh_part, double *__restrict__ fx_part, PlmGeom g, int m_tiles, int n_tiles,
                    int num_kb, int n_stages)
{
    constexpr int Q = 21;
    extern __shared__ unsigned char smem_dyn[];
    const TcSmem l = tc_smem_layout(smem_dyn);
    constexpr int stage_bytes = TC_A_BYTES + TF_B_BYTES + (SINGLE ? 0 : TF_B_BYTES);
    const int n_tile = blockIdx.x % n_tiles, m_tile = blockIdx.x / n_tiles;
    const int q = g.q;
    tc_init_barriers(l, n_stages);

    if (threadIdx.x < 128) {
        setmaxnreg_dec<TC_REG_PRODUCER>();
        if (threadIdx.x == 0) {
            const uint64_t keep = l2_policy_evict_last();
            int s = 0;
            uint32_t ph = 0;
            for (int kb = 0; kb < num_kb; kb++) {
                mbar_wait_bounded(&l.empty[s], ph ^ 1u);
                unsigned char *st = l.ring + s * stage_bytes;
                mbar_expect_tx(&l.full[s], (uint32_t)stage_bytes);
                tma_load_2d(st, &tm_x, kb * TC_BK, m_tile * TC_BM, &l.full[s]);
                tma_load_2d_hint(st + TC_A_BYTES, &tm_whi, kb * TC_BK, n_tile * TF_BN, &l.full[s], keep);
                if (!SINGLE)
                    tma_load_2d_hint(st + TC_A_BYTES + TF_B_BYTES, &tm_wlo, kb * TC_BK, n_tile * TF_BN, &l.full[s], keep);
                if (++s == n_stages) { s = 0; ph ^= 1u; }
            }
        }
        return;
    }
    setmaxnreg_inc<TC_REG_CONSUMER>();
    const int ct = threadIdx.x - 128;
    {
        const int cw = ct >> 7;
        const uint64_t arow = (uint64_t)((cw * 64 * TC_BK * 2) >> 4);
        constexpr uint64_t OFFH = (uint64_t)(TC_A_BYTES >> 4), OFFL = (uint64_t)((TC_A_BYTES + TF_B_BYTES) >> 4);
        float acc[TF_BN / 2];
#pragma unroll
        for (int u = 0; u < TF_BN / 2; u++) acc[u] = 0.f;
        int s = 0;
        uint32_t ph = 0;
        tc_mainloop<TF_BN>(acc, l.full, l.empty, s, ph, n_stages, stage_bytes, 0, num_kb, make_desc_sw128(l.ring),
                           arow, OFFH, arow, OFFL, !SINGLE);
        consumer_sync();
        float *stg = reinterpret_cast<float *>(l.ring);
        const int t = ct & 127;
        const int r0 = cw * 64 + (t >> 5) * 16 + ((t & 31) >> 2);
#pragma unroll
        for (int c8 = 0; c8 < TF_BN / 8; c8++) {
            const int col = 8 * c8 + 2 * (t & 3);
            stg[r0 * TF_PITCH + col] = acc[4 * c8];
            stg[r0 * TF_PITCH + col + 1] = acc[4 * c8 + 1];
            stg[(r0 + 8) * TF_PITCH + col] = acc[4 * c8 + 2];
            stg[(r0 + 8) * TF_PITCH + col + 1] = acc[4 * c8 + 3];
        }
        consumer_sync();
    }
    const float *stg = reinterpret_cast<const float *>(l.ring);
    const int ehalf = ct >> 7;
    const int r = ct & 127;
    const int quad = r >> 5, lane = r & 31;
    const int ntile_part = m_tiles * 4;
    const int64_t n = (int64_t)m_tile * TC_BM + r;
    const int64_t nc = n < g.N ? n : g.N - 1;
    const float wn = n < g.N ? wts[nc] : 0.f;
    const float *v = stg + r * TF_PITCH + ehalf * 88;
#pragma unroll
    for (int s = 0; s < 4; s++) {
        const int i = n_tile * TF_SITES + ehalf * 4 + s;
        if (i >= g.L) break;
        const int si = (int)((msa4[(int64_t)(i >> 2) * g.Nld + nc] >> (8 * (i & 3))) & 0xffu);
        const float w = si < q ? wn : 0.f;
        float z[Q];
        float mx = -INFINITY;
#pragma unroll
        for (int a = 0; a < Q; a++) {
            z[a] = (a < q) ? v[s * Q + a] + h[i * q + a] : -INFINITY;
            mx = fmaxf(mx, z[a]);
        }
        float zs = 0.f, sum = 0.f;
#pragma unroll
        for (int a = 0; a < Q; a++) {
            if (a == si) zs = z[a];
            z[a] = (a < q) ? expf(z[a] - mx) : 0.f;
            sum += z[a];
        }
        const double fx_local = (w == 0.f) ? 0.0 : -((double)w * (double)(zs - mx - logf(sum)));
        const float inv = w / sum;
        float *ghp = gh_part + ((int64_t)i * ntile_part + m_tile * 4 + quad) * g.S;
#pragma unroll
        for (int a = 0; a < Q; a++) {
            const float rr = z[a] * inv - (a == si ? w : 0.f);
            if (a < q) {
                if (n < g.N) {
                    const int64_t off = ((int64_t)i * q + a) * Kp + n;
                    const __nv_bfloat16 hi = __float2bfloat16_rn(rr);
                    Rt_hi[off] = hi;
                    if (!SINGLE) Rt_lo[off] = __float2bfloat16_rn(rr - __bfloat162float(hi));
                }
            }
            const float tot = warp_sum(rr);
            if (lane == 0) ghp[a] = (a < q) ? tot : 0.f;
        }
        const double fw = warp_sum(fx_local);
        if (lane == 0) fx_part[(int64_t)i * ntile_part + m_tile * 4 + quad] = fw;
    }
}

constexpr int EXP_SITES = 4;
constexpr int EXP_THREADS = 256;

template <bool PADDED>
__device__ __forceinline__ int64_t expand_row(int i, int a, int q)
{
    if (PADDED) return (int64_t)(i / TF_SITES) * TF_BN + ((i % TF_SITES) / 4) * 88 + (i % 4) * 21 + a;
    return (int64_t)i * q + a;
}

__device__ __forceinline__ void cp_async4(void *smem_dst, const void *gmem_src)
{
    asm volatile("cp.async.ca.shared.global [%0], [%1], 4;" ::"r"(smem_u32(smem_dst)), "l"(gmem_src) : "memory");
}
__device__ __forceinline__ void cp_async_wait_all() { asm volatile("cp.async.wait_all;" ::: "memory"); }

constexpr int EXP_STATIC_Q = 21;
static size_t exp_wide_smem(int q) { return (size_t)EXP_SITES * EXP_SITES * q * q * sizeof(float); }

template <bool PADDED, bool WIDE = false>
__global__ void __launch_bounds__(EXP_THREADS)
expand_tc_kernel(const float *__restrict__ x, __nv_bfloat16 *__restrict__ W_hi, __nv_bfloat16 *__restrict__ W_lo,
                 int L, int q, int64_t ldw, int single)
{
    __shared__ float sJ_static[WIDE ? 1 : EXP_SITES * EXP_SITES * EXP_STATIC_Q * EXP_STATIC_Q];
    extern __shared__ float sJ_dyn[];
    float *const sJ = WIDE ? sJ_dyn : sJ_static;
    const int ti = blockIdx.y, tj = blockIdx.x;
    if (tj < ti) return;
    const int i0 = ti * EXP_SITES, j0 = tj * EXP_SITES;
    const int ni = min(EXP_SITES, L - i0), nj = min(EXP_SITES, L - j0);
    const int qq = q * q;
    for (int ii = 0; ii < ni; ii++) {
        const int i = i0 + ii, jlo = max(j0, i + 1);
        if (jlo >= j0 + nj) continue;
        const float *src = x + (int64_t)L * q + ((int64_t)i * (2 * L - i - 1) / 2 + (jlo - i - 1)) * qq;
        float *dst = sJ + (ii * EXP_SITES + (jlo - j0)) * qq;
        const int n = (j0 + nj - jlo) * qq;
        for (int e = threadIdx.x; e < n; e += blockDim.x) cp_async4(dst + e, src + e);
    }
    cp_async_wait_all();
    __syncthreads();
    const int lane = threadIdx.x & 31, warp = threadIdx.x >> 5;
    auto write_tile = [&](int r0, int nr, int c0, int nc) {
        const int width = nc * q;
        int csite[4], colN[4], colT[4];
#pragma unroll
        for (int k = 0; k < 4; k++) {
            const int c = 2 * lane + 64 * (k >> 1) + (k & 1);
            const int cs = c / q, cb = c - cs * q;
            csite[k] = c0 + cs;
            colN[k] = cs * qq + cb;
            colT[k] = cs * EXP_SITES * qq + cb * q;
        }
        for (int rr = warp; rr < nr * q; rr += EXP_THREADS / 32) {
            const int rs = rr / q, ra = rr - rs * q, r = r0 + rs;
            const int rowN = rs * EXP_SITES * qq + ra * q, rowT = rs * qq + ra;
            const int64_t off = expand_row<PADDED>(r, ra, q) * ldw + (int64_t)c0 * q;
            auto elem = [&](int k) -> float {
                if (r < csite[k]) return sJ[rowN + colN[k]];
                if (r > csite[k]) return sJ[rowT + colT[k]];
                return 0.f;
            };
#pragma unroll
            for (int h = 0; h < 2; h++) {
                const int c = 2 * lane + 64 * h;
                if (c >= width) continue;
                const float v0 = elem(2 * h);
                const __nv_bfloat16 h0 = __float2bfloat16_rn(v0);
                const __nv_bfloat16 l0 = __float2bfloat16_rn(v0 - __bfloat162float(h0));
                if (c + 1 < width) {
                    const float v1 = elem(2 * h + 1);
                    const __nv_bfloat16 h1 = __float2bfloat16_rn(v1);
                    const __nv_bfloat16 l1 = __float2bfloat16_rn(v1 - __bfloat162float(h1));
                    *reinterpret_cast<__nv_bfloat162 *>(W_hi + off + c) = __halves2bfloat162(h0, h1);
                    if (!single) *reinterpret_cast<__nv_bfloat162 *>(W_lo + off + c) = __halves2bfloat162(l0, l1);
                } else {
                    W_hi[off + c] = h0;
                    if (!single) W_lo[off + c] = l0;
                }
            }
        }
    };
    write_tile(i0, ni, j0, nj);
    if (ti != tj) write_tile(j0, nj, i0, ni);
}

__global__ void build_x_kernel(const uint32_t *__restrict__ msa4, __nv_bfloat16 *__restrict__ X, int64_t n0,
                               int64_t nreal, int64_t Nld, int L, int q, int64_t ldx)
{
    const int64_t r = blockIdx.x;
    const bool real = r < nreal;
    for (int e = threadIdx.x; e < L * q; e += blockDim.x) {
        const int j = e / q, b = e - j * q;
        const int code = real ? (int)((msa4[(int64_t)(j >> 2) * Nld + n0 + r] >> (8 * (j & 3))) & 0xffu) : 255;
        X[r * ldx + e] = __float2bfloat16(code == b ? 1.0f : 0.0f);
    }
}

template <int Q, bool ONEHOT, bool RUNTIME_Q = false>
__global__ void __launch_bounds__(128)
plm_softmax_kernel(const float *__restrict__ Zt, int64_t ldz, const float *__restrict__ h,
                   const uint32_t *__restrict__ msa4, const float *__restrict__ wts,
                   __nv_bfloat16 *__restrict__ Rt_hi, __nv_bfloat16 *__restrict__ Rt_lo, int64_t Kp,
                   float *__restrict__ gh_part, double *__restrict__ fx_part, PlmGeom g, int ntiles, int64_t n_base)
{
    static_assert(Q <= 32, "s_gh holds 32 states per warp");
    const int q = RUNTIME_Q ? g.q : Q;
    __shared__ float s_gh[4 * 32];
    __shared__ double s_fx[4];
    const int tile = (int)(n_base >> 8) + blockIdx.x, i = blockIdx.y;
    const int tid = threadIdx.x, lane = tid & 31, warp = tid >> 5;
    const int64_t N = g.N;
    const int64_t nl = (int64_t)blockIdx.x * 256 + 2 * tid;
    const int64_t n0 = n_base + nl;
    const int64_t m0 = n0 < N ? n0 : ((N - 1) & ~(int64_t)1);
    const int64_t ml = m0 - n_base;
    const uint2 wi = *reinterpret_cast<const uint2 *>(msa4 + (int64_t)(i >> 2) * g.Nld + m0);
    const int sh = 8 * (i & 3);
    const int si[2] = {(int)((wi.x >> sh) & 0xffu), (int)((wi.y >> sh) & 0xffu)};
    float w[2];
    w[0] = (n0 < N && si[0] < q) ? wts[n0] : 0.f;
    w[1] = (n0 + 1 < N && si[1] < q) ? wts[n0 + 1] : 0.f;
    float z[2][Q];
    double fx_local = 0.0;
    if (ONEHOT) {
#pragma unroll
        for (int k = 0; k < 2; k++)
#pragma unroll
            for (int a = 0; a < Q; a++) z[k][a] = (a == si[k]) ? w[k] : 0.f;
    } else {
        float mx[2] = {-INFINITY, -INFINITY};
#pragma unroll
        for (int a = 0; a < Q; a++) {
            if (a < q) {
                const float2 v = *reinterpret_cast<const float2 *>(Zt + ((int64_t)i * q + a) * ldz + ml);
                const float ha = h[i * q + a];
                z[0][a] = v.x + ha;
                z[1][a] = v.y + ha;
                mx[0] = fmaxf(mx[0], z[0][a]);
                mx[1] = fmaxf(mx[1], z[1][a]);
            } else {
                z[0][a] = -INFINITY;
                z[1][a] = -INFINITY;
            }
        }
#pragma unroll
        for (int k = 0; k < 2; k++) {
            float zs = 0.f, sum = 0.f;
#pragma unroll
            for (int a = 0; a < Q; a++) {
                if (a == si[k]) zs = z[k][a];
                z[k][a] = a < q ? expf(z[k][a] - mx[k]) : 0.f;
                sum += z[k][a];
            }
            if (w[k] != 0.f) fx_local -= (double)w[k] * (double)(zs - mx[k] - logf(sum));
            const float inv = w[k] / sum;
#pragma unroll
            for (int a = 0; a < Q; a++) z[k][a] = z[k][a] * inv - (a == si[k] ? w[k] : 0.f);
        }
    }
#pragma unroll
    for (int a = 0; a < Q; a++) {
        if (a >= q) break;
        if (n0 < N) {
            const int64_t off = ((int64_t)i * q + a) * Kp + nl;
            const __nv_bfloat162 hi = __floats2bfloat162_rn(z[0][a], z[1][a]);
            *reinterpret_cast<__nv_bfloat162 *>(Rt_hi + off) = hi;
            if (Rt_lo != nullptr)
                *reinterpret_cast<__nv_bfloat162 *>(Rt_lo + off) =
                    __floats2bfloat162_rn(z[0][a] - __low2float(hi), z[1][a] - __high2float(hi));
        }
        const float v = warp_sum(z[0][a] + z[1][a]);
        if (lane == 0) s_gh[warp * 32 + a] = v;
    }
    const double fw = warp_sum(fx_local);
    if (lane == 0) s_fx[warp] = fw;
    __syncthreads();
    if (tid < g.S) {
        float tot = 0.f;
        if (tid < q)
            for (int ww = 0; ww < 4; ww++) tot += s_gh[ww * 32 + tid];
        gh_part[((int64_t)i * ntiles + tile) * g.S + tid] = tot;
    }
    if (tid == 0) fx_part[(int64_t)i * ntiles + tile] = (s_fx[0] + s_fx[1]) + (s_fx[2] + s_fx[3]);
}

__global__ void build_xt_kernel(const uint32_t *__restrict__ msa4, __nv_bfloat16 *__restrict__ Xt, int64_t n0,
                                int64_t N, int64_t Nld, int64_t Kp, int L, int q)
{
    const int64_t n = (int64_t)blockIdx.x * blockDim.x + threadIdx.x;
    const int j = blockIdx.y;
    if (n >= Kp) return;
    int code = 255;
    if (n0 + n < N) code = (int)((msa4[(int64_t)(j >> 2) * Nld + n0 + n] >> (8 * (j & 3))) & 0xffu);
    for (int b = 0; b < q; b++)
        Xt[((int64_t)j * q + b) * Kp + n] = __float2bfloat16(code == b ? 1.0f : 0.0f);
}

constexpr int FIN_SITES = 4;
constexpr int FIN_W = FIN_SITES * 21;
constexpr int FIN_PITCH = FIN_W + 1;
constexpr int FIN_THREADS = 256;
constexpr int FIN_SMEM = 2 * FIN_W * FIN_PITCH * (int)sizeof(float);
constexpr int FIN_BATCH = 8;
static int fin_pitch(int q) { return q <= 21 ? FIN_PITCH : FIN_SITES * q + 1; }
static int fin_smem_bytes(int q) { return q <= 21 ? FIN_SMEM : 2 * (fin_pitch(q) - 1) * fin_pitch(q) * (int)sizeof(float); }

template <bool WIDE = false>
__global__ void __launch_bounds__(FIN_THREADS)
finalize_pairs_tc_kernel(const float *__restrict__ Gd, int planes, int64_t plane, float *__restrict__ gJ, int L,
                         int q, int Np, float scale, int wide_pitch)
{
    const int pitch = WIDE ? wide_pitch : FIN_PITCH;
    extern __shared__ float fin_smem[];
    float *sA = fin_smem;
    float *sB = fin_smem + (pitch - 1) * pitch;
    const int ti = blockIdx.y, tj = blockIdx.x;
    if (tj < ti) return;
    const int i0 = ti * FIN_SITES, j0 = tj * FIN_SITES;
    const int wi = min(FIN_SITES, L - i0) * q, wj = min(FIN_SITES, L - j0) * q;
    auto stage = [&](float *dst, int row0, int rows, int col0, int cols) {
        const int V = (cols % 4 == 0) ? 4 : 1;
        const int nv = cols / V;
        const int dr = FIN_THREADS / nv, dc = FIN_THREADS - dr * nv;
        int r = threadIdx.x / nv, c = threadIdx.x - r * nv;
        while (r < rows) {
            float4 v[FIN_BATCH];
            int off[FIN_BATCH];
#pragma unroll
            for (int u = 0; u < FIN_BATCH; u++) {
                off[u] = r < rows ? r * pitch + c * V : -1;
                if (r < rows) {
                    const float *p = Gd + (int64_t)(row0 + r) * Np + (col0 + c * V);
                    v[u] = V == 4 ? *reinterpret_cast<const float4 *>(p) : make_float4(p[0], 0.f, 0.f, 0.f);
#pragma unroll
                    for (int s = 1; s < TC_MAX_KSPLIT; s++) {
                        if (s >= planes) break;
                        const float *ps = p + s * plane;
                        const float4 w = V == 4 ? *reinterpret_cast<const float4 *>(ps) : make_float4(ps[0], 0.f, 0.f, 0.f);
                        v[u].x += w.x; v[u].y += w.y; v[u].z += w.z; v[u].w += w.w;
                    }
                }
                c += dc; r += dr;
                if (c >= nv) { c -= nv; r++; }
            }
#pragma unroll
            for (int u = 0; u < FIN_BATCH; u++) {
                if (off[u] < 0) break;
                float *d = dst + off[u];
                d[0] = v[u].x;
                if (V == 4) { d[1] = v[u].y; d[2] = v[u].z; d[3] = v[u].w; }
            }
        }
    };
    stage(sA, i0 * q, wi, j0 * q, wj);
    stage(sB, j0 * q, wj, i0 * q, wi);
    __syncthreads();
    const int qq = q * q;
    const int sj = FIN_THREADS / qq, sa = (FIN_THREADS % qq) / q, sb = FIN_THREADS % q;
    for (int ii = 0; ii * q < wi; ii++) {
        const int i = i0 + ii, jlo = max(j0, i + 1);
        const int n = (j0 + wj / q - jlo) * qq;
        if (n <= 0) continue;
        float *out = gJ + ((int64_t)i * (2 * L - i - 1) / 2 + (jlo - i - 1)) * qq;
        int jj = jlo - j0 + threadIdx.x / qq, a = (threadIdx.x % qq) / q, b = threadIdx.x % q;
        for (int e = threadIdx.x; e < n; e += FIN_THREADS) {
            const float v1 = sB[(jj * q + b) * pitch + ii * q + a];
            const float v2 = sA[(ii * q + a) * pitch + jj * q + b];
            out[e] = scale * (v1 + v2);
            b += sb; a += sa; jj += sj;
            if (b >= q) { b -= q; a++; }
            if (a >= q) { a -= q; jj++; }
        }
    }
}

static int env_int_once(const char *name, int *cache)
{
    if (*cache == -2) {
        const char *e = getenv(name);
        *cache = e ? atoi(e) : -1;
    }
    return *cache;
}

static int stages_for(int stage_bytes)
{
    return std::max(2, std::min(TC_MAX_STAGES, (TC_SMEM_LIMIT - TC_SMEM_HEAD) / stage_bytes));
}

typedef CUresult (*PFN_encodeTiled)(CUtensorMap *, CUtensorMapDataType, cuuint32_t, void *, const cuuint64_t *,
                                    const cuuint64_t *, const cuuint32_t *, const cuuint32_t *, CUtensorMapInterleave,
                                    CUtensorMapSwizzle, CUtensorMapL2promotion, CUtensorMapFloatOOBfill);

static PFN_encodeTiled get_encode_fn()
{
    static PFN_encodeTiled fn = nullptr;
    if (fn) return fn;
    void *p = nullptr;
    cudaDriverEntryPointQueryResult qres;
    if (cudaGetDriverEntryPoint("cuTensorMapEncodeTiled", &p, cudaEnableDefault, &qres) != cudaSuccess ||
        qres != cudaDriverEntryPointSuccess || !p)
        return nullptr;
    fn = reinterpret_cast<PFN_encodeTiled>(p);
    return fn;
}

static int make_map(CUtensorMap *m, void *base, int64_t rows, int64_t kp, int box_rows)
{
    PFN_encodeTiled fn = get_encode_fn();
    if (!fn) { set_error("cuTensorMapEncodeTiled entry point not available"); return 1; }
    cuuint64_t gdim[2] = {(cuuint64_t)kp, (cuuint64_t)rows};
    cuuint64_t gstride[1] = {(cuuint64_t)kp * 2};
    cuuint32_t box[2] = {(cuuint32_t)TC_BK, (cuuint32_t)box_rows};
    cuuint32_t estr[2] = {1, 1};
    CUresult r = fn(m, CU_TENSOR_MAP_DATA_TYPE_BFLOAT16, 2, base, gdim, gstride, box, estr,
                    CU_TENSOR_MAP_INTERLEAVE_NONE, CU_TENSOR_MAP_SWIZZLE_128B, CU_TENSOR_MAP_L2_PROMOTION_L2_256B,
                    CU_TENSOR_MAP_FLOAT_OOB_FILL_NONE);
    if (r != CUDA_SUCCESS) { set_error("cuTensorMapEncodeTiled failed with code " + std::to_string((int)r)); return 1; }
    return 0;
}

static int backward_ksplit(int64_t tiles, int num_kb, int sm_count)
{
    static int ks_env = -2;
    const int e = env_int_once("EVC_KSPLIT", &ks_env);
    int ks = 1;
    if (e > 0) {
        ks = std::min(e, TC_MAX_KSPLIT);
    } else {
        double best = 0.0;
        for (int s = 1; s <= 4 && s <= num_kb; s++) {
            const int64_t units = tiles * s;
            const double eff = (double)units / ((double)sm_count * (double)ceil_div(units, sm_count));
            if (eff >= 0.97) { ks = s; break; }
            if (eff > best) { best = eff; ks = s; }
        }
    }
    ks = std::max(1, std::min(ks, num_kb));
    return (int)ceil_div(num_kb, ceil_div(num_kb, ks));
}

int64_t plm_seq_chunk_round(int64_t seq_chunk) { return seq_chunk <= 0 ? 0 : round_up(seq_chunk, PLM_SEQ_CHUNK_ALIGN); }

void plm_tc_geometry(const PlmGeom &g, int sm_count, int64_t seq_chunk, PlmTcGeom &t)
{
    const int64_t lq = (int64_t)g.L * g.q;
    const int64_t c = plm_seq_chunk_round(seq_chunk);
    t.C = (c == 0 || c >= g.N) ? g.N : c;
    t.n_chunks = (int)ceil_div(g.N, t.C);
    t.Mp = round_up(lq, TC_BM);
    t.Np = round_up(lq, TC_BN);
    t.Kp = round_up(t.C, TC_BK);
    const int64_t tiles = (t.Mp / TC_BM) * (t.Np / TC_BN);
    t.ksplit = backward_ksplit(tiles, (int)(t.Kp / TC_BK), sm_count);
    t.ksplit_last = backward_ksplit(tiles, (int)(t.kp_chunk(t.n_chunks - 1, g.N) / TC_BK), sm_count);
    t.planes = std::max(t.ksplit, t.ksplit_last);
}

int plm_tc_build_xt(const PlmGeom &g, const PlmTcGeom &t, const uint32_t *d_msa4, void *d_xt, int64_t n0,
                    cudaStream_t st)
{
    dim3 grid((unsigned)ceil_div(t.Kp, 256), (unsigned)g.L);
    build_xt_kernel<<<grid, 256, 0, st>>>(d_msa4, reinterpret_cast<__nv_bfloat16 *>(d_xt), n0, g.N, g.Nld, t.Kp,
                                          g.L, g.q);
    EVC_KERNEL_CHECK();
    return 0;
}

int plm_tc_make_maps(const PlmTcGeom &t, void *d_xt, void *d_rt_hi, void *d_rt_lo, void *maps_out)
{
    CUtensorMap *m = reinterpret_cast<CUtensorMap *>(maps_out);
    if (make_map(&m[0], d_xt, t.Mp, t.Kp, TC_BM)) return 1;
    if (make_map(&m[1], d_rt_hi, t.Np, t.Kp, TC_BN)) return 1;
    if (make_map(&m[2], d_rt_lo, t.Np, t.Kp, TC_BN)) return 1;
    return 0;
}

int plm_tc_backward(const PlmGeom &g, const PlmTcGeom &t, const void *maps, float *d_Gd, int single, int chunk,
                    cudaStream_t st)
{
    const CUtensorMap *m = reinterpret_cast<const CUtensorMap *>(maps);
    const int stage = TC_A_BYTES + TC_B_BYTES + (single ? 0 : TC_B_BYTES);
    const int n_stages = stages_for(stage);
    const size_t smem = (size_t)n_stages * stage + TC_SMEM_HEAD;
    static int kc_env = -2;
    const int kc = env_int_once("EVC_KCHUNK", &kc_env);
    const int k_chunk = kc > 0 ? kc : TC_K_CHUNK;
    const int m_tiles = (int)(t.Mp / TC_BM), n_tiles = (int)(t.Np / TC_BN);
    const bool last = chunk == t.n_chunks - 1;
    const int ksplit = last ? t.ksplit_last : t.ksplit;
    const int num_kb = (int)(t.kp_chunk(chunk, g.N) / TC_BK);
    const int grid = m_tiles * n_tiles * ksplit;
    const int64_t plane = t.Mp * t.Np;
    if (chunk == 0) {
        if (single) {
            EVC_CUDA(cudaFuncSetAttribute(tc_gemm_kernel<0, 1>, cudaFuncAttributeMaxDynamicSharedMemorySize, TC_SMEM_LIMIT));
            tc_gemm_kernel<0, 1><<<grid, TC_THREADS, smem, st>>>(m[0], m[1], m[2], d_Gd, t.Np, m_tiles, n_tiles,
                                                                num_kb, k_chunk, m_tiles, n_stages, ksplit, plane, 0);
        } else {
            EVC_CUDA(cudaFuncSetAttribute(tc_gemm_kernel<0, 0>, cudaFuncAttributeMaxDynamicSharedMemorySize, TC_SMEM_LIMIT));
            tc_gemm_kernel<0, 0><<<grid, TC_THREADS, smem, st>>>(m[0], m[1], m[2], d_Gd, t.Np, m_tiles, n_tiles,
                                                                num_kb, k_chunk, m_tiles, n_stages, ksplit, plane, 0);
        }
    } else {
        const int acc_planes = t.ksplit;
        if (single) {
            EVC_CUDA(cudaFuncSetAttribute(tc_gemm_kernel<0, 1, 1>, cudaFuncAttributeMaxDynamicSharedMemorySize, TC_SMEM_LIMIT));
            tc_gemm_kernel<0, 1, 1><<<grid, TC_THREADS, smem, st>>>(m[0], m[1], m[2], d_Gd, t.Np, m_tiles, n_tiles,
                                                                   num_kb, k_chunk, m_tiles, n_stages, ksplit, plane,
                                                                   acc_planes);
        } else {
            EVC_CUDA(cudaFuncSetAttribute(tc_gemm_kernel<0, 0, 1>, cudaFuncAttributeMaxDynamicSharedMemorySize, TC_SMEM_LIMIT));
            tc_gemm_kernel<0, 0, 1><<<grid, TC_THREADS, smem, st>>>(m[0], m[1], m[2], d_Gd, t.Np, m_tiles, n_tiles,
                                                                   num_kb, k_chunk, m_tiles, n_stages, ksplit, plane,
                                                                   acc_planes);
        }
    }
    EVC_KERNEL_CHECK();
    return 0;
}

int plm_tc_finalize_pairs(const PlmGeom &g, const PlmTcGeom &t, const float *d_Gd, int planes, float *d_gJ,
                          float scale, cudaStream_t st)
{
    const unsigned nt = (unsigned)ceil_div(g.L, FIN_SITES);
    auto kernel = g.q > 21 ? finalize_pairs_tc_kernel<true> : finalize_pairs_tc_kernel<false>;
    const int smem = fin_smem_bytes(g.q);
    EVC_CUDA(cudaFuncSetAttribute(kernel, cudaFuncAttributeMaxDynamicSharedMemorySize, smem));
    kernel<<<dim3(nt, nt), FIN_THREADS, smem, st>>>(d_Gd, planes, t.Mp * t.Np, d_gJ, g.L, g.q, (int)t.Np, scale,
                                                    fin_pitch(g.q));
    EVC_KERNEL_CHECK();
    return 0;
}

void plm_tcf_geometry(const PlmGeom &g, const PlmTcGeom &tc, PlmTcfGeom &t)
{
    const int64_t lq = (int64_t)g.L * g.q;
    t.Mp = round_up(lq, TC_BM);
    t.Kw = round_up(lq, TC_BK);
    t.Ns = round_up(tc.C, TC_BN);
    t.Xrows = round_up(tc.C, 384);
    t.ntiles_s = (int)ceil_div(g.N, 256);
}

int plm_tcf_build_x(const PlmGeom &g, const PlmTcfGeom &t, const uint32_t *d_msa4, void *d_x1h, int64_t n0,
                    cudaStream_t st)
{
    build_x_kernel<<<(unsigned)t.Xrows, 256, 0, st>>>(d_msa4, reinterpret_cast<__nv_bfloat16 *>(d_x1h), n0,
                                                    std::min(t.Xrows, g.N - n0), g.Nld, g.L, g.q, t.Kw);
    EVC_KERNEL_CHECK();
    return 0;
}

int plm_tcf_make_maps(const PlmTcfGeom &t, void *d_wt_hi, void *d_wt_lo, void *d_x1h, void *maps_out)
{
    CUtensorMap *m = reinterpret_cast<CUtensorMap *>(maps_out);
    if (make_map(&m[0], d_wt_hi, t.Mp, t.Kw, TC_BM)) return 1;
    if (make_map(&m[1], d_wt_lo, t.Mp, t.Kw, TC_BM)) return 1;
    if (make_map(&m[2], d_x1h, t.Xrows, t.Kw, TC_BN)) return 1;
    return 0;
}

int plm_tcf_expand(const PlmGeom &g, const PlmTcfGeom &t, const float *d_x, void *d_wt_hi, void *d_wt_lo,
                   int single, cudaStream_t st)
{
    const unsigned nt = (unsigned)ceil_div(g.L, EXP_SITES);
    if (g.q > EXP_STATIC_Q) {
        const size_t smem = exp_wide_smem(g.q);
        EVC_CUDA(cudaFuncSetAttribute(expand_tc_kernel<false, true>, cudaFuncAttributeMaxDynamicSharedMemorySize,
                                      (int)smem));
        expand_tc_kernel<false, true><<<dim3(nt, nt), EXP_THREADS, smem, st>>>(
            d_x, reinterpret_cast<__nv_bfloat16 *>(d_wt_hi), reinterpret_cast<__nv_bfloat16 *>(d_wt_lo), g.L, g.q,
            t.Kw, single);
        EVC_KERNEL_CHECK();
        return 0;
    }
    expand_tc_kernel<false><<<dim3(nt, nt), EXP_THREADS, 0, st>>>(d_x, reinterpret_cast<__nv_bfloat16 *>(d_wt_hi),
                                                                  reinterpret_cast<__nv_bfloat16 *>(d_wt_lo), g.L, g.q,
                                                                  t.Kw, single);
    EVC_KERNEL_CHECK();
    return 0;
}

static int forward_mgroup(const PlmTcfGeom &t, int single, int m_tiles)
{
    static int mg_env = -2;
    const int e = env_int_once("EVC_MGROUP", &mg_env);
    if (e > 0) return std::min(e, m_tiles);
    static int mb_env = -2;
    const int mb = env_int_once("EVC_MGROUP_MB", &mb_env);
    const double budget = (mb > 0 ? mb : 24) * 1.0e6;
    const double per_tile = (double)TC_BM * (double)t.Kw * 2.0 * (single ? 1.0 : 2.0);
    return std::max(1, std::min(m_tiles, (int)(budget / per_tile)));
}

int plm_tcf_logits(const PlmGeom &g, const PlmTcfGeom &t, const void *maps, float *d_zt, int single, int64_t nreal,
                   cudaStream_t st)
{
    const CUtensorMap *m = reinterpret_cast<const CUtensorMap *>(maps);
    const int stage = TC_A_BYTES + TC_B_BYTES + (single ? 0 : TC_A_BYTES);
    const int n_stages = stages_for(stage);
    const size_t smem = (size_t)n_stages * stage + TC_SMEM_HEAD;
    const int m_tiles = (int)(t.Mp / TC_BM), n_tiles = (int)ceil_div(nreal, TC_BN);
    const int num_kb = (int)(t.Kw / TC_BK);
    const int grid = m_tiles * n_tiles;
    const int kchunk = num_kb <= 128 ? num_kb : TC_K_CHUNK;
    const int mgroup = forward_mgroup(t, single, m_tiles);
    if (single) {
        EVC_CUDA(cudaFuncSetAttribute(tc_gemm_kernel<1, 1>, cudaFuncAttributeMaxDynamicSharedMemorySize, TC_SMEM_LIMIT));
        tc_gemm_kernel<1, 1><<<grid, TC_THREADS, smem, st>>>(m[0], m[1], m[2], d_zt, t.Ns, m_tiles, n_tiles, num_kb,
                                                            kchunk, mgroup, n_stages, 1, 0, 0);
    } else {
        EVC_CUDA(cudaFuncSetAttribute(tc_gemm_kernel<1, 0>, cudaFuncAttributeMaxDynamicSharedMemorySize, TC_SMEM_LIMIT));
        tc_gemm_kernel<1, 0><<<grid, TC_THREADS, smem, st>>>(m[0], m[1], m[2], d_zt, t.Ns, m_tiles, n_tiles, num_kb,
                                                            kchunk, mgroup, n_stages, 1, 0, 0);
    }
    EVC_KERNEL_CHECK();
    return 0;
}

template <bool ONEHOT>
static int launch_softmax(const PlmGeom &g, int ntiles, const float *d_zt, int64_t ldz, const float *d_x,
                          const uint32_t *d_msa4, const float *d_wts, __nv_bfloat16 *hi, __nv_bfloat16 *lo,
                          int64_t Kp, float *d_gh_part, double *d_fx_part, int64_t n0, int64_t nreal, cudaStream_t st)
{
    dim3 grid((unsigned)ceil_div(nreal, 256), (unsigned)g.L);
    switch (g.q) {
        case 21: plm_softmax_kernel<21, ONEHOT><<<grid, 128, 0, st>>>(d_zt, ldz, d_x, d_msa4, d_wts, hi, lo, Kp, d_gh_part, d_fx_part, g, ntiles, n0); break;
        case 20: plm_softmax_kernel<20, ONEHOT><<<grid, 128, 0, st>>>(d_zt, ldz, d_x, d_msa4, d_wts, hi, lo, Kp, d_gh_part, d_fx_part, g, ntiles, n0); break;
        case 5: plm_softmax_kernel<5, ONEHOT><<<grid, 128, 0, st>>>(d_zt, ldz, d_x, d_msa4, d_wts, hi, lo, Kp, d_gh_part, d_fx_part, g, ntiles, n0); break;
        case 4: plm_softmax_kernel<4, ONEHOT><<<grid, 128, 0, st>>>(d_zt, ldz, d_x, d_msa4, d_wts, hi, lo, Kp, d_gh_part, d_fx_part, g, ntiles, n0); break;
        default:
            if (g.q < 2 || g.q > PLM_MAX_Q) { set_error("plm softmax kernel: unsupported q"); return 1; }
            if (g.q <= 8)
                plm_softmax_kernel<8, ONEHOT, true><<<grid, 128, 0, st>>>(d_zt, ldz, d_x, d_msa4, d_wts, hi, lo, Kp, d_gh_part, d_fx_part, g, ntiles, n0);
            else if (g.q <= 16)
                plm_softmax_kernel<16, ONEHOT, true><<<grid, 128, 0, st>>>(d_zt, ldz, d_x, d_msa4, d_wts, hi, lo, Kp, d_gh_part, d_fx_part, g, ntiles, n0);
            else
                plm_softmax_kernel<32, ONEHOT, true><<<grid, 128, 0, st>>>(d_zt, ldz, d_x, d_msa4, d_wts, hi, lo, Kp, d_gh_part, d_fx_part, g, ntiles, n0);
    }
    EVC_KERNEL_CHECK();
    return 0;
}

int plm_tcf_softmax(const PlmGeom &g, const PlmTcfGeom &t, const float *d_zt, const float *d_x,
                    const uint32_t *d_msa4, const float *d_wts, void *d_rt_hi, void *d_rt_lo, int64_t Kp,
                    float *d_gh_part, double *d_fx_part, int64_t n0, int64_t nreal, cudaStream_t st)
{
    return launch_softmax<false>(g, t.ntiles_s, d_zt, t.Ns, d_x, d_msa4, d_wts,
                                 reinterpret_cast<__nv_bfloat16 *>(d_rt_hi), reinterpret_cast<__nv_bfloat16 *>(d_rt_lo),
                                 Kp, d_gh_part, d_fx_part, n0, nreal, st);
}

int plm_tc_onehot_residual(const PlmGeom &g, int ntiles, const uint32_t *d_msa4, const float *d_wts, void *d_rt_hi,
                           void *d_rt_lo, int64_t Kp, float *d_gh_part, double *d_fx_part, int64_t n0, int64_t nreal,
                           cudaStream_t st)
{
    return launch_softmax<true>(g, ntiles, nullptr, 0, nullptr, d_msa4, d_wts,
                                reinterpret_cast<__nv_bfloat16 *>(d_rt_hi), reinterpret_cast<__nv_bfloat16 *>(d_rt_lo),
                                Kp, d_gh_part, d_fx_part, n0, nreal, st);
}

void plm_tcff_geometry(const PlmGeom &g, PlmTcffGeom &t)
{
    t.n_tiles = (int)ceil_div(g.L, TF_SITES);
    t.Np = (int64_t)t.n_tiles * TF_BN;
    t.Kw = round_up((int64_t)g.L * g.q, TC_BK);
    t.m_tiles = (int)ceil_div(g.N, TC_BM);
    t.Xrows = round_up(g.N, 384);
    t.ntile_part = t.m_tiles * 4;
}

bool plm_tcff_supported(const PlmGeom &g) { return g.S == 21; }

int plm_tcff_make_maps(const PlmTcffGeom &t, void *d_x1h, void *d_wp_hi, void *d_wp_lo, void *maps_out)
{
    CUtensorMap *m = reinterpret_cast<CUtensorMap *>(maps_out);
    if (make_map(&m[0], d_x1h, t.Xrows, t.Kw, TC_BM)) return 1;
    if (make_map(&m[1], d_wp_hi, t.Np, t.Kw, TF_BN)) return 1;
    if (make_map(&m[2], d_wp_lo, t.Np, t.Kw, TF_BN)) return 1;
    return 0;
}

int plm_tcff_expand(const PlmGeom &g, const PlmTcffGeom &t, const float *d_x, void *d_wp_hi, void *d_wp_lo,
                    int single, cudaStream_t st)
{
    const unsigned nt = (unsigned)ceil_div(g.L, EXP_SITES);
    expand_tc_kernel<true><<<dim3(nt, nt), EXP_THREADS, 0, st>>>(d_x, reinterpret_cast<__nv_bfloat16 *>(d_wp_hi),
                                                                 reinterpret_cast<__nv_bfloat16 *>(d_wp_lo), g.L, g.q,
                                                                 t.Kw, single);
    EVC_KERNEL_CHECK();
    return 0;
}

int plm_tcff_forward(const PlmGeom &g, const PlmTcffGeom &t, const void *maps, const float *d_x,
                     const uint32_t *d_msa4, const float *d_wts, void *d_rt_hi, void *d_rt_lo, int64_t Kp,
                     float *d_gh_part, double *d_fx_part, int single, cudaStream_t st)
{
    const CUtensorMap *m = reinterpret_cast<const CUtensorMap *>(maps);
    const int stage = TC_A_BYTES + TF_B_BYTES + (single ? 0 : TF_B_BYTES);
    const int n_stages = stages_for(stage);
    const size_t smem = (size_t)n_stages * stage + TC_SMEM_HEAD;
    const int grid = t.m_tiles * t.n_tiles;
    auto kernel = single ? tc_fwd_fused_kernel<1> : tc_fwd_fused_kernel<0>;
    EVC_CUDA(cudaFuncSetAttribute(kernel, cudaFuncAttributeMaxDynamicSharedMemorySize, TC_SMEM_LIMIT));
    kernel<<<grid, TC_THREADS, smem, st>>>(m[0], m[1], m[2], d_x, d_msa4, d_wts, reinterpret_cast<__nv_bfloat16 *>(d_rt_hi),
                                           reinterpret_cast<__nv_bfloat16 *>(d_rt_lo), Kp, d_gh_part, d_fx_part, g,
                                           t.m_tiles, t.n_tiles, (int)(t.Kw / TC_BK), n_stages);
    EVC_KERNEL_CHECK();
    return 0;
}

size_t plm_tc_map_bytes() { return 3 * sizeof(CUtensorMap); }

}
```

### include/evcplm.h

```cpp
#ifndef EVCPLM_H
#define EVCPLM_H

#include <stdint.h>

#ifdef __cplusplus
extern "C" {
#endif

#define EVCPLM_ABI_VERSION 2

typedef struct evc_plm evc_plm_t;

int evc_abi_version(void);
const char *evc_last_error(void);
int evc_device_count(void);
int evc_device_info(int32_t device, int32_t *sm_count, int32_t *cc_major, int32_t *cc_minor,
                    int64_t *total_mem_bytes);

int evc_hamming_counts(const uint8_t *codes, int64_t N, int32_t L, int32_t min_identical,
                       int32_t device, int32_t *counts_out);

int64_t evc_hamming_plane_words(int64_t N, int32_t L);
int64_t evc_hamming_num_tiles(int64_t N);
int evc_hamming_pack(const uint8_t *d_codes, int64_t N, int32_t L, uint32_t *d_planes, void *stream);
int evc_hamming_count_tiles(const uint32_t *d_planes, int64_t N, int32_t L, int32_t min_identical,
                            int64_t tile_begin, int64_t tile_end, int32_t *d_counts ,
                            void *stream);

int evc_hamming_counts_mult(const uint8_t *codes, const int32_t *mult, int64_t N, int32_t L, int32_t min_identical,
                            int32_t device, int32_t *counts_out);
int evc_hamming_count_tiles_mult(const uint32_t *d_planes, const int32_t *d_mult, int64_t N, int32_t L,
                                 int32_t min_identical, int64_t tile_begin, int64_t tile_end,
                                 int32_t *d_counts , void *stream);

int evc_msa_unique(const uint8_t *d_codes , int64_t N, int32_t L, int32_t *d_first, int32_t *d_inverse,
                   int32_t *d_mult, int64_t *U_out, void *stream);
int evc_msa_unique_host(const uint8_t *codes , int64_t N, int32_t L, int32_t device, int32_t *first_out,
                        int32_t *inverse_out, int32_t *mult_out, int64_t *U_out);

int evc_identities_to_seq(const uint8_t *d_codes , const uint8_t *d_seq , int64_t N, int32_t L,
                          int32_t *d_out, void *stream);

int evc_a2m_scan(const char *path, int64_t *n_rows, int64_t *width, int64_t *ids_bytes);
int evc_a2m_read(const char *path, int64_t n_rows, int64_t width, uint8_t *raw, char *ids, int64_t ids_bytes);
int evc_msa_encode(const uint8_t *raw, int64_t n_rows, int64_t width, const uint8_t *lut, const int64_t *cols,
                   int64_t n_cols, uint8_t *valid_out, uint8_t *codes_out, int64_t *n_valid_out);

int evc_plm_create(evc_plm_t **out, const uint8_t *codes , int64_t N, int32_t L,
                   int32_t q, int32_t gap_code ,
                   const float *weights , int32_t device);
int evc_plm_create_alphabet(evc_plm_t **out, const uint8_t *codes , int64_t N, int32_t L,
                            int32_t q, int32_t gap_code ,
                            const float *weights , int32_t device);
void evc_plm_destroy(evc_plm_t *h);
int64_t evc_plm_num_params(const evc_plm_t *h);

int evc_plm_eval_data(evc_plm_t *h, const float *d_x, float *d_g, double *d_fx, void *stream);

int evc_plm_set_backward(evc_plm_t *h, int32_t mode);
int evc_plm_set_forward(evc_plm_t *h, int32_t mode);

int evc_plm_set_precision(evc_plm_t *h, int32_t mode);

int evc_plm_set_seq_chunk(evc_plm_t *h, int64_t seq_chunk);
int evc_plm_tc_bytes(int64_t N, int32_t L, int32_t q, int32_t gap_code, int64_t seq_chunk, int32_t sm_count,
                     int64_t *bytes_out);
int evc_plm_tc_bytes_alphabet(int64_t N, int32_t L, int32_t q, int32_t gap_code, int64_t seq_chunk,
                              int32_t sm_count, int64_t *bytes_out);
int64_t evc_plm_device_bytes(const evc_plm_t *h);
int64_t evc_fit_workspace_bytes(int64_t n, int32_t m);
int evc_plm_set_host_history(evc_plm_t *h, int32_t host_pairs);
int evc_fit_workspace_split_bytes(int64_t n, int32_t m, int32_t host_pairs, int64_t *device_bytes,
                                  int64_t *host_bytes);
int evc_plm_host_bytes(const evc_plm_t *h, int64_t *bytes_out, double *pin_seconds_out);

int evc_plm_set_profiling(evc_plm_t *h, int32_t enable);
int evc_plm_last_stage_ms(evc_plm_t *h, float *ms_out);

int evc_plm_add_regulariser(evc_plm_t *h, const float *d_x, float *d_g, double *d_fx,
                            float lambda_h, float lambda_J, void *stream);

int evc_plm_eval_host(evc_plm_t *h, const float *x, float *g, double *fx_out,
                      float lambda_h, float lambda_J);

int evc_plm_weighted_counts(evc_plm_t *h, float *d_fi_counts, float *d_fij_counts, void *stream);

enum {
    EVC_LBFGS_SUCCESS = 0,
    EVC_LBFGS_ALREADY_MINIMIZED = 2,
    EVC_LBFGSERR_CANCELED = -1021,
    EVC_LBFGSERR_INVALIDPARAMETERS = -1000,
    EVC_LBFGSERR_MINIMUMSTEP = -1001,
    EVC_LBFGSERR_MAXIMUMSTEP = -1002,
    EVC_LBFGSERR_MAXIMUMLINESEARCH = -1003,
    EVC_LBFGSERR_MAXIMUMITERATION = -1004,
    EVC_LBFGSERR_WIDTHTOOSMALL = -1005,
    EVC_LBFGSERR_ROUNDING_ERROR = -1006,
    EVC_LBFGSERR_INCREASEGRADIENT = -1007
};
typedef struct {
    int32_t max_iterations;
    int32_t m;
    float epsilon;
    float lambda_h, lambda_J;
    int32_t max_linesearch;
    double min_step, max_step, ftol, gtol, xtol;
    int32_t precision_schedule;
    float switch_factor;
} evc_fit_params_t;
typedef struct {
    int32_t status;
    int32_t iterations;
    int32_t evaluations;
    int32_t switched_at;
    double fx, negloglk;
    double seconds;
} evc_fit_result_t;
typedef int (*evc_allreduce_cb)(void *user, float *d_buf, int64_t count, void *stream);
typedef int (*evc_progress_cb)(void *user, int32_t iteration, double fx, double xnorm, double gnorm, double step,
                               int32_t linesearch_evals, double negloglk, double hnorm, double enorm);
void evc_fit_default_params(evc_fit_params_t *p);
int evc_plm_fit(evc_plm_t *h, float *d_x, const evc_fit_params_t *params, evc_allreduce_cb allreduce,
                void *allreduce_user, evc_progress_cb progress, void *progress_user, evc_fit_result_t *result,
                void *stream);

#define EVC_FIT_STATE_VERSION 1
typedef struct {
    int32_t version;
    int32_t returning;
    int32_t status;
    int32_t k;
    int32_t evaluations;
    int32_t m, hist, end;
    int32_t low;
    int32_t switched_at;
    int64_t n;
    double fx, negloglk, xnorm, gnorm;
    double ys[32];
    double yy;
    double seconds;
} evc_fit_state_t;
typedef int (*evc_checkpoint_cb)(void *user, const evc_fit_state_t *state, void *stream);
int evc_plm_fit_checkpointed(evc_plm_t *h, float *d_x, const evc_fit_params_t *params, evc_allreduce_cb allreduce,
                             void *allreduce_user, evc_progress_cb progress, void *progress_user,
                             evc_checkpoint_cb checkpoint, void *checkpoint_user, double checkpoint_interval,
                             const evc_fit_state_t *resume, evc_fit_result_t *result, void *stream);
int evc_plm_fit_prepare(evc_plm_t *h, int32_t m);
enum { EVC_FIT_VEC_X = 0, EVC_FIT_VEC_G = 1, EVC_FIT_VEC_S = 2, EVC_FIT_VEC_Y = 3 };
int evc_plm_fit_vector(evc_plm_t *h, int32_t which, int32_t slot, float **ptr_out);

int evc_plm_pack_fx(const double *d_fx, float *d_limbs, void *stream);
int evc_plm_unpack_fx(const float *d_limbs, double *d_fx, void *stream);

int evc_vec_dot(const float *d_a, const float *d_b, int64_t n, double *d_out, void *stream);
int evc_vec_axpby(float *d_y, const float *d_x, float a, float b, int64_t n, void *stream);
int evc_vec_copy(float *d_dst, const float *d_src, int64_t n, void *stream);
int evc_vec_sub(float *d_out, const float *d_a, const float *d_b, int64_t n, void *stream);
int evc_vec_checksum(const float *d_v, int64_t n, uint64_t *d_out, void *stream);
int evc_lbfgs_direction(float *d_d, const float *d_g, const float *d_S, const float *d_Y,
                        const double *d_ys, double *d_scratch, int64_t n, int32_t m,
                        int32_t bound, int32_t end, void *stream);
int evc_lbfgs_update_pair(float *d_S_slot, float *d_Y_slot, const float *d_x, const float *d_xp,
                          const float *d_g, const float *d_gp, double *d_ys_slot, double *d_yy,
                          int64_t n, void *stream);

int evc_ec_scores(const float *d_J_tri, const float *d_fij_tri, const float *d_fi, int32_t L, int32_t q,
                  float *d_fn_raw, float *d_fn_zero_sum, float *d_mi, void *stream);
int evc_plm_energies(evc_plm_t *h, const float *d_x, double *d_out, void *stream);

int evc_fn_scores(const float *d_J_tri, int32_t L, int32_t q, float *d_fn , void *stream);

#ifdef __cplusplus
}
#endif
#endif
```

Baseline: 4516 billion.

## Use 2:4 sparse WGMMA for forward logits with cluster-multicast weight tiles

The forward logits GEMM now treats the one-hot sequence operand as a 2:4 structured-sparse A matrix. A new packed fragment-plus-metadata layout is built per chunk, and the work goes to a new sparse wgmma kernel (m64n192k32.sp) instead of the dense SPLIT_A path. Weight tiles are split in halves and multicast across a 2-CTA cluster, so each CTA loads only half from global memory. The aim is to halve tensor-core K work and shrink operand traffic. The costs are a new packing kernel, cluster synchronisation overhead, and a removed dense template path. A host copy helper for the one-hot buffer is also added.

```diff
diff --git a/evcouplings_b200/_lib.py b/evcouplings_b200/_lib.py
--- a/evcouplings_b200/_lib.py
+++ b/evcouplings_b200/_lib.py
@@ -86,6 +86,7 @@
     "evc_plm_tc_bytes": (ctypes.c_int, [c_i64, c_i32, c_i32, c_i32, c_i64, c_i32, c_void_p]),
     "evc_plm_tc_bytes_alphabet": (ctypes.c_int, [c_i64, c_i32, c_i32, c_i32, c_i64, c_i32, c_void_p]),
     "evc_plm_device_bytes": (c_i64, [c_void_p]),
+    "evc_plm_copy_onehot": (ctypes.c_int, [c_void_p, c_void_p, c_i64]),
     "evc_fit_workspace_bytes": (c_i64, [c_i64, c_i32]),
     "evc_plm_set_host_history": (ctypes.c_int, [c_void_p, c_i32]),
     "evc_fit_workspace_split_bytes": (ctypes.c_int, [c_i64, c_i32, c_i32, c_void_p, c_void_p]),
diff --git a/evcouplings_b200/csrc/api.cu b/evcouplings_b200/csrc/api.cu
--- a/evcouplings_b200/csrc/api.cu
+++ b/evcouplings_b200/csrc/api.cu
@@ -437,9 +437,9 @@
         if (plm_tcf_expand(g, h->tcf, d_x, h->d_wt_hi, h->d_wt_lo, single, st)) return 1;
         for (int c = 0; c < h->tc.n_chunks; c++) {
             const int64_t n0 = (int64_t)c * h->tc.C, nreal = std::min(h->tc.C, g.N - n0);
-            if (plm_tcf_build_x(g, h->tcf, h->d_msa4, h->d_x1h, n0, st)) return 1;
+            if (plm_tcf_build_xsp(g, h->tcf, h->d_msa4, h->d_x1h, n0, st)) return 1;
             if (plm_tc_build_xt(g, h->tc, h->d_msa4, h->d_xt, n0, st)) return 1;
-            if (plm_tcf_logits(g, h->tcf, h->tcf_maps, h->d_zt, single, nreal, st)) return 1;
+            if (plm_tcf_logits(g, h->tcf, h->tcf_maps, h->d_x1h, h->d_zt, single, nreal, st)) return 1;
             if (plm_tcf_softmax(g, h->tcf, h->d_zt, d_x, h->d_msa4, h->d_wts, h->d_rt_hi, rt_lo, h->tc.Kp,
                                 h->d_gh_part2, h->d_fx_part2, n0, nreal, st))
                 return 1;
@@ -469,7 +469,7 @@
     } else if (tcf) {
         if (plm_tcf_expand(g, h->tcf, d_x, h->d_wt_hi, h->d_wt_lo, single, st)) return 1;
         if (prof) EVC_CUDA(cudaEventRecord(h->ev[1], st));
-        if (plm_tcf_logits(g, h->tcf, h->tcf_maps, h->d_zt, single, g.N, st)) return 1;
+        if (plm_tcf_logits(g, h->tcf, h->tcf_maps, h->d_x1h, h->d_zt, single, g.N, st)) return 1;
         if (prof) EVC_CUDA(cudaEventRecord(h->ev[2], st));
         if (plm_tcf_softmax(g, h->tcf, h->d_zt, d_x, h->d_msa4, h->d_wts, h->d_rt_hi, rt_lo, h->tc.Kp,
                             h->d_gh_part2, h->d_fx_part2, 0, g.N, st))
@@ -563,8 +563,13 @@
                 return 1;
             }
             EVC_CUDA(cudaMemset(h->d_x1h, 0, b.x));
-            if (h->tc.n_chunks == 1 && plm_tcf_build_x(h->g, t, h->d_msa4, h->d_x1h, 0, 0)) return 1;
+        }
+        if (h->tc.n_chunks == 1 && h->x1h_form != mode) {
+            if (mode == 1 ? plm_tcf_build_xsp(h->g, h->tcf, h->d_msa4, h->d_x1h, 0, 0)
+                          : plm_tcf_build_x(h->g, h->tcf, h->d_msa4, h->d_x1h, 0, 0))
+                return 1;
             EVC_CUDA(cudaDeviceSynchronize());
+            h->x1h_form = mode;
         }
     }
     if (mode == 1 && !h->d_zt) {
@@ -580,7 +585,7 @@
         EVC_CUDA(cudaMemset(h->d_wt_lo, 0, b.wt));
         h->tcf_maps = aligned_alloc(64, round_up((int64_t)plm_tc_map_bytes(), 64));
         if (!h->tcf_maps) { set_error("evc_plm_set_forward: out of host memory"); return 1; }
-        if (plm_tcf_make_maps(t, h->d_wt_hi, h->d_wt_lo, h->d_x1h, h->tcf_maps)) return 1;
+        if (plm_tcf_make_maps(t, h->d_wt_hi, h->d_wt_lo, h->tcf_maps)) return 1;
     }
     if (mode == 2 && !h->d_wp_hi) {
         plm_tcff_geometry(h->g, h->tcff);
@@ -663,6 +668,21 @@
 }
 
 int64_t evc_plm_device_bytes(const evc_plm_t *h) { return h ? h->bytes + fit_work_bytes(h->fit) : -1; }
+
+int evc_plm_copy_onehot(const evc_plm_t *h, void *host_dst, int64_t bytes)
+{
+    if (!h || !host_dst) { set_error("evc_plm_copy_onehot: null pointer"); return 1; }
+    if (!h->d_x1h) { set_error("evc_plm_copy_onehot: the handle has no tensor-core forward (evc_plm_set_forward)"); return 1; }
+    const int64_t have = h->tcf.Xrows * h->tcf.Kw * 2;
+    if (bytes != have) {
+        set_error("evc_plm_copy_onehot: bytes must be the operand's allocation, " + std::to_string(have));
+        return 1;
+    }
+    EVC_CUDA(cudaSetDevice(h->device));
+    EVC_CUDA(cudaDeviceSynchronize());
+    EVC_CUDA(cudaMemcpy(host_dst, h->d_x1h, (size_t)bytes, cudaMemcpyDeviceToHost));
+    return 0;
+}
 
 int64_t evc_fit_workspace_bytes(int64_t n, int32_t m) { return n > 0 && m > 0 ? fit_work_bytes(n, m) : -1; }
 
diff --git a/evcouplings_b200/csrc/internal.h b/evcouplings_b200/csrc/internal.h
--- a/evcouplings_b200/csrc/internal.h
+++ b/evcouplings_b200/csrc/internal.h
@@ -97,11 +97,13 @@
 void plm_tcf_geometry(const PlmGeom &g, const PlmTcGeom &tc, PlmTcfGeom &t);
 int plm_tcf_build_x(const PlmGeom &g, const PlmTcfGeom &t, const uint32_t *d_msa4, void *d_x1h, int64_t n0,
                     cudaStream_t st);
-int plm_tcf_make_maps(const PlmTcfGeom &t, void *d_wt_hi, void *d_wt_lo, void *d_x1h, void *maps_out_host);
+int plm_tcf_build_xsp(const PlmGeom &g, const PlmTcfGeom &t, const uint32_t *d_msa4, void *d_x1h, int64_t n0,
+                      cudaStream_t st);
+int plm_tcf_make_maps(const PlmTcfGeom &t, void *d_wt_hi, void *d_wt_lo, void *maps_out_host);
 int plm_tcf_expand(const PlmGeom &g, const PlmTcfGeom &t, const float *d_x, void *d_wt_hi, void *d_wt_lo,
                    int single, cudaStream_t st);
-int plm_tcf_logits(const PlmGeom &g, const PlmTcfGeom &t, const void *maps_host, float *d_zt, int single,
-                   int64_t nreal, cudaStream_t st);
+int plm_tcf_logits(const PlmGeom &g, const PlmTcfGeom &t, const void *maps_host, const void *d_x1h, float *d_zt,
+                   int single, int64_t nreal, cudaStream_t st);
 int plm_tcf_softmax(const PlmGeom &g, const PlmTcfGeom &t, const float *d_zt, const float *d_x,
                     const uint32_t *d_msa4, const float *d_wts, void *d_rt_hi, void *d_rt_lo, int64_t Kp,
                     float *d_gh_part, double *d_fx_part, int64_t n0, int64_t nreal, cudaStream_t st);
@@ -180,6 +182,7 @@
     int fwd_mode = 0;
     evc::PlmTcfGeom tcf{};
     void *d_x1h = nullptr;
+    int x1h_form = 0;
     void *d_wt_hi = nullptr;
     void *d_wt_lo = nullptr;
     float *d_zt = nullptr;
diff --git a/evcouplings_b200/csrc/plm_tc.cu b/evcouplings_b200/csrc/plm_tc.cu
--- a/evcouplings_b200/csrc/plm_tc.cu
+++ b/evcouplings_b200/csrc/plm_tc.cu
@@ -161,6 +161,74 @@
         : "l"(da), "l"(db), "r"(scale_d));
 }
 
+__device__ __forceinline__ void wgmma_sp_bf16_192(float *d, const uint4 &a, uint32_t e, uint64_t db, uint32_t scale_d)
+{
+    asm volatile(
+        "{\n.reg .pred p;\n"
+        "setp.ne.b32 p, %102, 0;\n"
+        "wgmma.mma_async.sp.sync.aligned.m64n192k32.f32.bf16.bf16 "
+        "{"
+        "%0, %1, %2, %3, %4, %5, %6, %7, %8, %9, %10, %11, %12, %13, %14, %15, "
+        "%16, %17, %18, %19, %20, %21, %22, %23, %24, %25, %26, %27, %28, %29, %30, %31, "
+        "%32, %33, %34, %35, %36, %37, %38, %39, %40, %41, %42, %43, %44, %45, %46, %47, "
+        "%48, %49, %50, %51, %52, %53, %54, %55, %56, %57, %58, %59, %60, %61, %62, %63, "
+        "%64, %65, %66, %67, %68, %69, %70, %71, %72, %73, %74, %75, %76, %77, %78, %79, "
+        "%80, %81, %82, %83, %84, %85, %86, %87, %88, %89, %90, %91, %92, %93, %94, %95"
+        "}, {%96, %97, %98, %99}, %100, %101, 0, p, 1, 1, 0;\n}\n"
+        : "+f"(d[0]), "+f"(d[1]), "+f"(d[2]), "+f"(d[3]), "+f"(d[4]), "+f"(d[5]), "+f"(d[6]), "+f"(d[7]),
+          "+f"(d[8]), "+f"(d[9]), "+f"(d[10]), "+f"(d[11]), "+f"(d[12]), "+f"(d[13]), "+f"(d[14]), "+f"(d[15]),
+          "+f"(d[16]), "+f"(d[17]), "+f"(d[18]), "+f"(d[19]), "+f"(d[20]), "+f"(d[21]), "+f"(d[22]), "+f"(d[23]),
+          "+f"(d[24]), "+f"(d[25]), "+f"(d[26]), "+f"(d[27]), "+f"(d[28]), "+f"(d[29]), "+f"(d[30]), "+f"(d[31]),
+          "+f"(d[32]), "+f"(d[33]), "+f"(d[34]), "+f"(d[35]), "+f"(d[36]), "+f"(d[37]), "+f"(d[38]), "+f"(d[39]),
+          "+f"(d[40]), "+f"(d[41]), "+f"(d[42]), "+f"(d[43]), "+f"(d[44]), "+f"(d[45]), "+f"(d[46]), "+f"(d[47]),
+          "+f"(d[48]), "+f"(d[49]), "+f"(d[50]), "+f"(d[51]), "+f"(d[52]), "+f"(d[53]), "+f"(d[54]), "+f"(d[55]),
+          "+f"(d[56]), "+f"(d[57]), "+f"(d[58]), "+f"(d[59]), "+f"(d[60]), "+f"(d[61]), "+f"(d[62]), "+f"(d[63]),
+          "+f"(d[64]), "+f"(d[65]), "+f"(d[66]), "+f"(d[67]), "+f"(d[68]), "+f"(d[69]), "+f"(d[70]), "+f"(d[71]),
+          "+f"(d[72]), "+f"(d[73]), "+f"(d[74]), "+f"(d[75]), "+f"(d[76]), "+f"(d[77]), "+f"(d[78]), "+f"(d[79]),
+          "+f"(d[80]), "+f"(d[81]), "+f"(d[82]), "+f"(d[83]), "+f"(d[84]), "+f"(d[85]), "+f"(d[86]), "+f"(d[87]),
+          "+f"(d[88]), "+f"(d[89]), "+f"(d[90]), "+f"(d[91]), "+f"(d[92]), "+f"(d[93]), "+f"(d[94]), "+f"(d[95])
+        : "r"(a.x), "r"(a.y), "r"(a.z), "r"(a.w), "l"(db), "r"(e), "r"(scale_d));
+}
+
+__device__ __forceinline__ uint4 lds128(uint32_t addr)
+{
+    uint4 v;
+    asm volatile("ld.shared.v4.u32 {%0, %1, %2, %3}, [%4];" : "=r"(v.x), "=r"(v.y), "=r"(v.z), "=r"(v.w) : "r"(addr));
+    return v;
+}
+__device__ __forceinline__ uint32_t lds32(uint32_t addr)
+{
+    uint32_t v;
+    asm volatile("ld.shared.u32 %0, [%1];" : "=r"(v) : "r"(addr));
+    return v;
+}
+__device__ __forceinline__ uint32_t cluster_ctarank()
+{
+    uint32_t r;
+    asm volatile("mov.u32 %0, %%cluster_ctarank;" : "=r"(r));
+    return r;
+}
+__device__ __forceinline__ void cluster_sync()
+{
+    asm volatile("barrier.cluster.arrive.release;\nbarrier.cluster.wait.acquire;" ::: "memory");
+}
+__device__ __forceinline__ void mbar_arrive_cluster(uint64_t *bar, uint32_t rank)
+{
+    uint32_t remote;
+    asm volatile("mapa.shared::cluster.u32 %0, %1, %2;" : "=r"(remote) : "r"(smem_u32(bar)), "r"(rank));
+    asm volatile("mbarrier.arrive.shared::cluster.b64 _, [%0];" ::"r"(remote) : "memory");
+}
+__device__ __forceinline__ void tma_load_2d_multicast(void *smem_dst, const CUtensorMap *tmap, int c0, int c1,
+                                                      uint64_t *bar, uint16_t mask, uint64_t policy)
+{
+    asm volatile(
+        "cp.async.bulk.tensor.2d.shared::cluster.global.mbarrier::complete_tx::bytes.multicast::cluster.L2::cache_hint"
+        " [%0], [%1, {%4, %5}], [%2], %3, %6;"
+        ::"r"(smem_u32(smem_dst)), "l"(reinterpret_cast<uint64_t>(tmap)), "r"(smem_u32(bar)), "h"(mask), "r"(c0),
+        "r"(c1), "l"(policy)
+        : "memory");
+}
+
 template <int N>
 __device__ __forceinline__ void wgmma_kblock(float *acc, uint64_t a, uint64_t b, uint64_t a2, uint64_t b2, bool two,
                                              bool overwrite)
@@ -236,7 +304,7 @@
     __syncthreads();
 }
 
-template <int SPLIT_A, int SINGLE, int ACC = 0>
+template <int SINGLE, int ACC = 0>
 __global__ void __launch_bounds__(TC_THREADS, 1)
 tc_gemm_kernel(const __grid_constant__ CUtensorMap tm0, const __grid_constant__ CUtensorMap tm1,
                const __grid_constant__ CUtensorMap tm2, float *__restrict__ D, int64_t ldd, int m_tiles, int n_tiles,
@@ -244,7 +312,7 @@
 {
     constexpr int BYTES0 = TC_A_BYTES;
     constexpr int BYTES1 = TC_B_BYTES;
-    constexpr int BYTES2 = SPLIT_A ? TC_A_BYTES : TC_B_BYTES;
+    constexpr int BYTES2 = TC_B_BYTES;
     constexpr int stage_bytes = BYTES0 + BYTES1 + (SINGLE ? 0 : BYTES2);
     extern __shared__ unsigned char smem_dyn[];
     const TcSmem l = tc_smem_layout(smem_dyn);
@@ -259,22 +327,15 @@
     if (threadIdx.x < 128) {
         setmaxnreg_dec<TC_REG_PRODUCER>();
         if (threadIdx.x == 0) {
-            const uint64_t keep = l2_policy_evict_last();
             int s = 0;
             uint32_t ph = 0;
             for (int kb = kb_begin; kb < kb_end; kb++) {
                 mbar_wait_bounded(&l.empty[s], ph ^ 1u);
                 unsigned char *st = l.ring + s * stage_bytes;
                 mbar_expect_tx(&l.full[s], (uint32_t)stage_bytes);
-                if (SPLIT_A) {
-                    tma_load_2d_hint(st, &tm0, kb * TC_BK, m_tile * TC_BM, &l.full[s], keep);
-                    tma_load_2d(st + BYTES0, &tm2, kb * TC_BK, n_tile * TC_BN, &l.full[s]);
-                    if (!SINGLE) tma_load_2d_hint(st + BYTES0 + BYTES1, &tm1, kb * TC_BK, m_tile * TC_BM, &l.full[s], keep);
-                } else {
-                    tma_load_2d(st, &tm0, kb * TC_BK, m_tile * TC_BM, &l.full[s]);
-                    tma_load_2d(st + BYTES0, &tm1, kb * TC_BK, n_tile * TC_BN, &l.full[s]);
-                    if (!SINGLE) tma_load_2d(st + BYTES0 + BYTES1, &tm2, kb * TC_BK, n_tile * TC_BN, &l.full[s]);
-                }
+                tma_load_2d(st, &tm0, kb * TC_BK, m_tile * TC_BM, &l.full[s]);
+                tma_load_2d(st + BYTES0, &tm1, kb * TC_BK, n_tile * TC_BN, &l.full[s]);
+                if (!SINGLE) tma_load_2d(st + BYTES0 + BYTES1, &tm2, kb * TC_BK, n_tile * TC_BN, &l.full[s]);
                 if (++s == n_stages) { s = 0; ph ^= 1u; }
             }
         }
@@ -292,10 +353,8 @@
         uint32_t ph = 0;
         for (int c = 0; c < n_chunks; c++) {
             const int kb0 = kb_begin + c * k_chunk, kb1 = min(kb_end, kb0 + k_chunk);
-            if (SPLIT_A) tc_mainloop<TC_BN>(acc, l.full, l.empty, s, ph, n_stages, stage_bytes, kb0, kb1, desc0,
-                                            arow, OFF1, OFF2 + arow, OFF1, !SINGLE);
-            else tc_mainloop<TC_BN>(acc, l.full, l.empty, s, ph, n_stages, stage_bytes, kb0, kb1, desc0,
-                                    arow, OFF1, arow, OFF2, !SINGLE);
+            tc_mainloop<TC_BN>(acc, l.full, l.empty, s, ph, n_stages, stage_bytes, kb0, kb1, desc0,
+                               arow, OFF1, arow, OFF2, !SINGLE);
 #pragma unroll
             for (int u = 0; u < TC_BN / 2; u++) sum[u] = (c == 0) ? acc[u] : sum[u] + acc[u];
         }
@@ -319,6 +378,176 @@
             __stcs(reinterpret_cast<float2 *>(out + 8 * ldd + 8 * c8), make_float2(sum[4 * c8 + 2], sum[4 * c8 + 3]));
         }
     }
+}
+
+constexpr int XSP_STEP_BYTES = 2560;
+constexpr int XSP_KB_BYTES = 4 * XSP_STEP_BYTES;
+constexpr int SP_W_HALF = (TC_BN / 2) * TC_BK * 2;
+
+template <int SINGLE>
+__global__ void __launch_bounds__(TC_THREADS, 1)
+tc_sparse_logits_kernel(const __grid_constant__ CUtensorMap tm_hi, const __grid_constant__ CUtensorMap tm_lo,
+                        const unsigned char *__restrict__ xsp, float *__restrict__ Zt, int64_t ldz, int64_t rows_z,
+                        int state_tiles, int seq_tiles, int seq_units, int num_kb, int k_chunk, int group,
+                        int n_stages)
+{
+    constexpr int OFF_A = TC_B_BYTES;
+    constexpr int OFF_LO = TC_B_BYTES + XSP_KB_BYTES;
+    constexpr int stage_bytes = OFF_LO + (SINGLE ? 0 : TC_B_BYTES);
+    extern __shared__ unsigned char smem_dyn[];
+    const TcSmem l = tc_smem_layout(smem_dyn);
+    uint32_t cs;
+    asm volatile("mov.u32 %0, %%cluster_nctarank;" : "=r"(cs));
+    const uint32_t rank = cluster_ctarank();
+    int n_tile, unit;
+    decode_tile((int)(blockIdx.x / cs), state_tiles, seq_units, group, n_tile, unit);
+    const int seq_tile = unit * (int)cs + (int)rank;
+    const bool pad = seq_tile >= seq_tiles;
+    if (threadIdx.x == 0) {
+        for (int s = 0; s < n_stages; s++) {
+            mbar_init(&l.full[s], 1);
+            mbar_init(&l.empty[s], 8 * cs);
+        }
+        mbar_fence_init();
+    }
+    cluster_sync();
+
+    if (threadIdx.x < 128) {
+        setmaxnreg_dec<TC_REG_PRODUCER>();
+        if (threadIdx.x == 0) {
+            const uint64_t keep = l2_policy_evict_last();
+            const unsigned char *src = xsp + (int64_t)(pad ? 0 : seq_tile) * num_kb * XSP_KB_BYTES;
+            const int row0 = n_tile * TC_BN;
+            int s = 0;
+            uint32_t ph = 0;
+            for (int kb = 0; kb < num_kb; kb++) {
+                mbar_wait_bounded(&l.empty[s], ph ^ 1u);
+                unsigned char *st = l.ring + s * stage_bytes;
+                mbar_expect_tx(&l.full[s], (uint32_t)stage_bytes);
+                bulk_g2s(st + OFF_A, src + (int64_t)kb * XSP_KB_BYTES, XSP_KB_BYTES, &l.full[s]);
+                if (cs == 1) {
+                    for (int h = 0; h < 2; h++) {
+                        tma_load_2d_hint(st + h * SP_W_HALF, &tm_hi, kb * TC_BK, row0 + h * (TC_BN / 2), &l.full[s], keep);
+                        if (!SINGLE)
+                            tma_load_2d_hint(st + OFF_LO + h * SP_W_HALF, &tm_lo, kb * TC_BK, row0 + h * (TC_BN / 2),
+                                             &l.full[s], keep);
+                    }
+                } else {
+                    const int h = (int)rank;
+                    tma_load_2d_multicast(st + h * SP_W_HALF, &tm_hi, kb * TC_BK, row0 + h * (TC_BN / 2), &l.full[s],
+                                          (uint16_t)0x3, keep);
+                    if (!SINGLE)
+                        tma_load_2d_multicast(st + OFF_LO + h * SP_W_HALF, &tm_lo, kb * TC_BK, row0 + h * (TC_BN / 2),
+                                              &l.full[s], (uint16_t)0x3, keep);
+                }
+                if (++s == n_stages) { s = 0; ph ^= 1u; }
+            }
+        }
+    } else {
+        setmaxnreg_inc<TC_REG_CONSUMER>();
+        const int cw = (threadIdx.x >> 7) - 1;
+        const int t = threadIdx.x & 127;
+        const uint32_t a_addr = smem_u32(l.ring) + OFF_A + cw * 2 * XSP_STEP_BYTES + 16 * t;
+        const uint32_t e_addr = a_addr + 2048 - 12 * t;
+        const uint64_t desc0 = make_desc_sw128(l.ring);
+        constexpr uint64_t DLO = (uint64_t)(OFF_LO >> 4), DK32 = (uint64_t)((32 * 2) >> 4);
+        auto release = [&](int st) {
+            if ((threadIdx.x & 31) == 0) {
+                mbar_arrive_cluster(&l.empty[st], 0);
+                if (cs == 2) mbar_arrive_cluster(&l.empty[st], 1);
+            }
+        };
+        float acc[TC_BN / 2], sum[TC_BN / 2];
+#pragma unroll
+        for (int u = 0; u < TC_BN / 2; u++) acc[u] = 0.f;
+        const int n_chunks = (num_kb + k_chunk - 1) / k_chunk;
+        int s = 0;
+        uint32_t ph = 0;
+        for (int c = 0; c < n_chunks; c++) {
+            const int kb0 = c * k_chunk, kb1 = min(num_kb, kb0 + k_chunk);
+            for (int kb = kb0; kb < kb1; kb++) {
+                mbar_wait_bounded(&l.full[s], ph);
+                const uint32_t so = (uint32_t)(s * stage_bytes);
+                const uint4 a0 = lds128(a_addr + so), a1 = lds128(a_addr + so + XSP_STEP_BYTES);
+                const uint32_t e0 = lds32(e_addr + so), e1 = lds32(e_addr + so + XSP_STEP_BYTES);
+                wgmma_fence();
+                const uint64_t d = desc0 + (uint64_t)((s * stage_bytes) >> 4);
+                wgmma_sp_bf16_192(acc, a0, e0, d, kb == kb0 ? 0u : 1u);
+                if (!SINGLE) wgmma_sp_bf16_192(acc, a0, e0, d + DLO, 1u);
+                wgmma_sp_bf16_192(acc, a1, e1, d + DK32, 1u);
+                if (!SINGLE) wgmma_sp_bf16_192(acc, a1, e1, d + DLO + DK32, 1u);
+                wgmma_commit();
+                wgmma_wait<0>();
+                release(s);
+                if (++s == n_stages) { s = 0; ph ^= 1u; }
+            }
+            fence_regs<TC_BN / 2>(acc);
+#pragma unroll
+            for (int u = 0; u < TC_BN / 2; u++) sum[u] = (c == 0) ? acc[u] : sum[u] + acc[u];
+        }
+        if (!pad) {
+            const int64_t seq0 = (int64_t)seq_tile * TC_BM + cw * 64 + (t >> 5) * 16 + ((t & 31) >> 2);
+            const int64_t st0 = (int64_t)n_tile * TC_BN + 2 * (t & 3);
+#pragma unroll
+            for (int c8 = 0; c8 < TC_BN / 8; c8++)
+#pragma unroll
+                for (int e = 0; e < 4; e++) {
+                    const int64_t row = st0 + 8 * c8 + (e & 1), col = seq0 + 8 * (e >> 1);
+                    if (row < rows_z && col < ldz) __stcs(Zt + row * ldz + col, sum[4 * c8 + e]);
+                }
+        }
+    }
+    cluster_sync();
+}
+
+__device__ __forceinline__ uint32_t xsp_group(const uint32_t *__restrict__ msa4, int64_t Nld, int64_t n, bool real,
+                                              int k, int lq, int q, uint32_t &vals)
+{
+    uint32_t mask = 0;
+    if (real) {
+#pragma unroll
+        for (int p = 0; p < 4; p++) {
+            const int kk = k + p;
+            if (kk >= lq) break;
+            const int j = kk / q, b = kk - j * q;
+            const int code = (int)((msa4[(int64_t)(j >> 2) * Nld + n] >> (8 * (j & 3))) & 0xffu);
+            mask |= (uint32_t)(code == b) << p;
+        }
+    }
+    int i0 = 0, i1 = 1;
+    if (__popc(mask) == 2) { i0 = __ffs(mask) - 1; i1 = 31 - __clz(mask); }
+    else if (mask > 2) i1 = __ffs(mask) - 1;
+    vals = (((mask >> i0) & 1u) ? 0x3F80u : 0u) | ((((mask >> i1) & 1u) ? 0x3F80u : 0u) << 16);
+    return (uint32_t)(i0 | (i1 << 2));
+}
+
+__global__ void build_xsp_kernel(const uint32_t *__restrict__ msa4, unsigned char *__restrict__ out, int64_t n0,
+                                 int64_t nreal, int64_t Nld, int L, int q, int num_kb, int64_t n_frag)
+{
+    const int64_t gt = (int64_t)blockIdx.x * blockDim.x + threadIdx.x;
+    if (gt >= n_frag * 128) return;
+    const int64_t ci = gt >> 7;
+    const int t = (int)(gt & 127);
+    const int step = (int)(ci & 1), cw = (int)((ci >> 1) & 1);
+    const int64_t tkb = ci >> 2;
+    const int kb = (int)(tkb % num_kb);
+    const int64_t T = tkb / num_kb;
+    const int64_t r0 = T * TC_BM + cw * 64 + (t >> 5) * 16 + ((t & 31) >> 2), r1 = r0 + 8;
+    const int k0 = kb * TC_BK + step * 32, lq = L * q;
+    const int c = t & 3, h = c & 1;
+    uint32_t e = 0, v[2][2], unused;
+#pragma unroll
+    for (int rr = 0; rr < 2; rr++) {
+        const int64_t r = rr ? r1 : r0;
+#pragma unroll
+        for (int i = 0; i < 4; i++)
+            e |= xsp_group(msa4, Nld, n0 + r, r < nreal, k0 + 4 * (4 * h + i), lq, q, unused) << (16 * rr + 4 * i);
+#pragma unroll
+        for (int u = 0; u < 2; u++) xsp_group(msa4, Nld, n0 + r, r < nreal, k0 + 4 * (4 * u + c), lq, q, v[rr][u]);
+    }
+    unsigned char *frag = out + ci * XSP_STEP_BYTES;
+    reinterpret_cast<uint4 *>(frag)[t] = make_uint4(v[0][0], v[1][0], v[0][1], v[1][1]);
+    reinterpret_cast<uint32_t *>(frag + 2048)[t] = e;
 }
 
 constexpr int TF_BN = 176;
@@ -837,24 +1066,24 @@
     const int64_t plane = t.Mp * t.Np;
     if (chunk == 0) {
         if (single) {
-            EVC_CUDA(cudaFuncSetAttribute(tc_gemm_kernel<0, 1>, cudaFuncAttributeMaxDynamicSharedMemorySize, TC_SMEM_LIMIT));
-            tc_gemm_kernel<0, 1><<<grid, TC_THREADS, smem, st>>>(m[0], m[1], m[2], d_Gd, t.Np, m_tiles, n_tiles,
+            EVC_CUDA(cudaFuncSetAttribute(tc_gemm_kernel<1>, cudaFuncAttributeMaxDynamicSharedMemorySize, TC_SMEM_LIMIT));
+            tc_gemm_kernel<1><<<grid, TC_THREADS, smem, st>>>(m[0], m[1], m[2], d_Gd, t.Np, m_tiles, n_tiles,
                                                                 num_kb, k_chunk, m_tiles, n_stages, ksplit, plane, 0);
         } else {
-            EVC_CUDA(cudaFuncSetAttribute(tc_gemm_kernel<0, 0>, cudaFuncAttributeMaxDynamicSharedMemorySize, TC_SMEM_LIMIT));
-            tc_gemm_kernel<0, 0><<<grid, TC_THREADS, smem, st>>>(m[0], m[1], m[2], d_Gd, t.Np, m_tiles, n_tiles,
+            EVC_CUDA(cudaFuncSetAttribute(tc_gemm_kernel<0>, cudaFuncAttributeMaxDynamicSharedMemorySize, TC_SMEM_LIMIT));
+            tc_gemm_kernel<0><<<grid, TC_THREADS, smem, st>>>(m[0], m[1], m[2], d_Gd, t.Np, m_tiles, n_tiles,
                                                                 num_kb, k_chunk, m_tiles, n_stages, ksplit, plane, 0);
         }
     } else {
         const int acc_planes = t.ksplit;
         if (single) {
-            EVC_CUDA(cudaFuncSetAttribute(tc_gemm_kernel<0, 1, 1>, cudaFuncAttributeMaxDynamicSharedMemorySize, TC_SMEM_LIMIT));
-            tc_gemm_kernel<0, 1, 1><<<grid, TC_THREADS, smem, st>>>(m[0], m[1], m[2], d_Gd, t.Np, m_tiles, n_tiles,
+            EVC_CUDA(cudaFuncSetAttribute(tc_gemm_kernel<1, 1>, cudaFuncAttributeMaxDynamicSharedMemorySize, TC_SMEM_LIMIT));
+            tc_gemm_kernel<1, 1><<<grid, TC_THREADS, smem, st>>>(m[0], m[1], m[2], d_Gd, t.Np, m_tiles, n_tiles,
                                                                    num_kb, k_chunk, m_tiles, n_stages, ksplit, plane,
                                                                    acc_planes);
         } else {
-            EVC_CUDA(cudaFuncSetAttribute(tc_gemm_kernel<0, 0, 1>, cudaFuncAttributeMaxDynamicSharedMemorySize, TC_SMEM_LIMIT));
-            tc_gemm_kernel<0, 0, 1><<<grid, TC_THREADS, smem, st>>>(m[0], m[1], m[2], d_Gd, t.Np, m_tiles, n_tiles,
+            EVC_CUDA(cudaFuncSetAttribute(tc_gemm_kernel<0, 1>, cudaFuncAttributeMaxDynamicSharedMemorySize, TC_SMEM_LIMIT));
+            tc_gemm_kernel<0, 1><<<grid, TC_THREADS, smem, st>>>(m[0], m[1], m[2], d_Gd, t.Np, m_tiles, n_tiles,
                                                                    num_kb, k_chunk, m_tiles, n_stages, ksplit, plane,
                                                                    acc_planes);
         }
@@ -895,12 +1124,23 @@
     return 0;
 }
 
-int plm_tcf_make_maps(const PlmTcfGeom &t, void *d_wt_hi, void *d_wt_lo, void *d_x1h, void *maps_out)
+int plm_tcf_make_maps(const PlmTcfGeom &t, void *d_wt_hi, void *d_wt_lo, void *maps_out)
 {
     CUtensorMap *m = reinterpret_cast<CUtensorMap *>(maps_out);
-    if (make_map(&m[0], d_wt_hi, t.Mp, t.Kw, TC_BM)) return 1;
-    if (make_map(&m[1], d_wt_lo, t.Mp, t.Kw, TC_BM)) return 1;
-    if (make_map(&m[2], d_x1h, t.Xrows, t.Kw, TC_BN)) return 1;
+    if (make_map(&m[0], d_wt_hi, t.Mp, t.Kw, TC_BN / 2)) return 1;
+    if (make_map(&m[1], d_wt_lo, t.Mp, t.Kw, TC_BN / 2)) return 1;
+    return 0;
+}
+
+int plm_tcf_build_xsp(const PlmGeom &g, const PlmTcfGeom &t, const uint32_t *d_msa4, void *d_x1h, int64_t n0,
+                      cudaStream_t st)
+{
+    const int num_kb = (int)(t.Kw / TC_BK);
+    const int64_t n_frag = t.Xrows / TC_BM * num_kb * 4;
+    build_xsp_kernel<<<(unsigned)ceil_div(n_frag * 128, 256), 256, 0, st>>>(
+        d_msa4, reinterpret_cast<unsigned char *>(d_x1h), n0, std::min(t.Xrows, g.N - n0), g.Nld, g.L, g.q, num_kb,
+        n_frag);
+    EVC_KERNEL_CHECK();
     return 0;
 }
 
@@ -925,39 +1165,54 @@
     return 0;
 }
 
-static int forward_mgroup(const PlmTcfGeom &t, int single, int m_tiles)
+static int forward_group(const PlmTcfGeom &t, int single, int tiles)
 {
     static int mg_env = -2;
     const int e = env_int_once("EVC_MGROUP", &mg_env);
-    if (e > 0) return std::min(e, m_tiles);
+    if (e > 0) return std::min(e, tiles);
     static int mb_env = -2;
     const int mb = env_int_once("EVC_MGROUP_MB", &mb_env);
     const double budget = (mb > 0 ? mb : 24) * 1.0e6;
-    const double per_tile = (double)TC_BM * (double)t.Kw * 2.0 * (single ? 1.0 : 2.0);
-    return std::max(1, std::min(m_tiles, (int)(budget / per_tile)));
-}
-
-int plm_tcf_logits(const PlmGeom &g, const PlmTcfGeom &t, const void *maps, float *d_zt, int single, int64_t nreal,
-                   cudaStream_t st)
+    const double per_tile = (double)TC_BN * (double)t.Kw * 2.0 * (single ? 1.0 : 2.0);
+    return std::max(1, std::min(tiles, (int)(budget / per_tile)));
+}
+
+static int forward_cluster()
+{
+    static int cl_env = -2;
+    const int e = env_int_once("EVC_FWD_CLUSTER", &cl_env);
+    return e == 1 ? 1 : 2;
+}
+
+int plm_tcf_logits(const PlmGeom &g, const PlmTcfGeom &t, const void *maps, const void *d_x1h, float *d_zt,
+                   int single, int64_t nreal, cudaStream_t st)
 {
     const CUtensorMap *m = reinterpret_cast<const CUtensorMap *>(maps);
-    const int stage = TC_A_BYTES + TC_B_BYTES + (single ? 0 : TC_A_BYTES);
+    const int stage = TC_B_BYTES + XSP_KB_BYTES + (single ? 0 : TC_B_BYTES);
     const int n_stages = stages_for(stage);
     const size_t smem = (size_t)n_stages * stage + TC_SMEM_HEAD;
-    const int m_tiles = (int)(t.Mp / TC_BM), n_tiles = (int)ceil_div(nreal, TC_BN);
+    const int cs = forward_cluster();
+    const int state_tiles = (int)ceil_div((int64_t)g.L * g.q, TC_BN);
+    const int seq_tiles = (int)ceil_div(nreal, TC_BM), seq_units = (int)ceil_div(seq_tiles, cs);
     const int num_kb = (int)(t.Kw / TC_BK);
-    const int grid = m_tiles * n_tiles;
     const int kchunk = num_kb <= 128 ? num_kb : TC_K_CHUNK;
-    const int mgroup = forward_mgroup(t, single, m_tiles);
-    if (single) {
-        EVC_CUDA(cudaFuncSetAttribute(tc_gemm_kernel<1, 1>, cudaFuncAttributeMaxDynamicSharedMemorySize, TC_SMEM_LIMIT));
-        tc_gemm_kernel<1, 1><<<grid, TC_THREADS, smem, st>>>(m[0], m[1], m[2], d_zt, t.Ns, m_tiles, n_tiles, num_kb,
-                                                            kchunk, mgroup, n_stages, 1, 0, 0);
-    } else {
-        EVC_CUDA(cudaFuncSetAttribute(tc_gemm_kernel<1, 0>, cudaFuncAttributeMaxDynamicSharedMemorySize, TC_SMEM_LIMIT));
-        tc_gemm_kernel<1, 0><<<grid, TC_THREADS, smem, st>>>(m[0], m[1], m[2], d_zt, t.Ns, m_tiles, n_tiles, num_kb,
-                                                            kchunk, mgroup, n_stages, 1, 0, 0);
-    }
+    const int group = forward_group(t, single, state_tiles);
+    auto kernel = single ? tc_sparse_logits_kernel<1> : tc_sparse_logits_kernel<0>;
+    EVC_CUDA(cudaFuncSetAttribute(kernel, cudaFuncAttributeMaxDynamicSharedMemorySize, TC_SMEM_LIMIT));
+    cudaLaunchConfig_t cfg = {};
+    cfg.gridDim = dim3((unsigned)(state_tiles * seq_units * cs));
+    cfg.blockDim = dim3(TC_THREADS);
+    cfg.dynamicSmemBytes = smem;
+    cfg.stream = st;
+    cudaLaunchAttribute attr[1];
+    attr[0].id = cudaLaunchAttributeClusterDimension;
+    attr[0].val.clusterDim.x = (unsigned)cs;
+    attr[0].val.clusterDim.y = 1;
+    attr[0].val.clusterDim.z = 1;
+    cfg.attrs = attr;
+    cfg.numAttrs = 1;
+    EVC_CUDA(cudaLaunchKernelEx(&cfg, kernel, m[0], m[1], reinterpret_cast<const unsigned char *>(d_x1h), d_zt, t.Ns,
+                                t.Mp, state_tiles, seq_tiles, seq_units, num_kb, kchunk, group, n_stages));
     EVC_KERNEL_CHECK();
     return 0;
 }
diff --git a/include/evcplm.h b/include/evcplm.h
--- a/include/evcplm.h
+++ b/include/evcplm.h
@@ -68,6 +68,7 @@
 int evc_plm_tc_bytes_alphabet(int64_t N, int32_t L, int32_t q, int32_t gap_code, int64_t seq_chunk,
                               int32_t sm_count, int64_t *bytes_out);
 int64_t evc_plm_device_bytes(const evc_plm_t *h);
+int evc_plm_copy_onehot(const evc_plm_t *h, void *host_dst, int64_t bytes);
 int64_t evc_fit_workspace_bytes(int64_t n, int32_t m);
 int evc_plm_set_host_history(evc_plm_t *h, int32_t host_pairs);
 int evc_fit_workspace_split_bytes(int64_t n, int32_t m, int32_t host_pairs, int64_t *device_bytes,
```

Result: faster. 4881 billion, median of 6 (+8.1%).
